# Wx-Alliance-Alliance-Meteo/paradis_model

Hardware: AMD Instinct MI355X
Metric: training samples/sec (whole node) on 5.625° ERA5 grid, 1/2/4/8 MI355X (higher is better)
Workload: dtype f32; 1 GPU; era5_5.625deg_32x64_S1_B32; grid=32x64, rollout_steps=1, per_gpu_batch=32, global_batch=32, parameters=60038475, optimizer=adamw, parallelism=dp1, gemm_arithmetic=bf16x3, mode=train, hip_graph=False, activation_checkpointing=False

## Files before the change

### paradis_model_amd/csrc/gemm_common.h

```cpp
#pragma once
#include <algorithm>
#include <cstdlib>
#include <initializer_list>
#include "common.h"

struct GemmArgs {
  const float* A; const float* B; float* C;
  int M, N, K;
  int64_t lda, ldb, ldc;
  int64_t a_bs, b_bs, c_bs;
  int nbatch;
  int inner;
  int64_t a_is, b_is;
  const float* bias; const float* map; const float* res; const float* zmul; float* zout;
  const float* gate;
  int64_t res_bs, zmul_bs, zout_bs;
  int act;
  int stagger;
  float* rowsum;
  const float* m8; const float* pw; int cin;
  const uint32_t* a_amax; const uint32_t* b_amax;
  int io16;
};

enum class WgradKind { Staged, Dma, Bf16x3, F16x2, Amp128, Tall, Square };
struct WgradWorkspace {
  int S, M, K;
  size_t rowsum_offset() const { return (size_t)S * M * K; }
  size_t bytes() const { return (size_t)S * M * ((size_t)K + 1) * sizeof(float) + 256; }
  float* rowsums(void* ws) const { return (float*)ws + rowsum_offset(); }
};

struct WgradPlan {
  WgradKind kind;
  int S;
  int grid, block;
  size_t lds;
  bool fused_rowsums;
  bool to_slabs;
  WgradWorkspace ws;
};

struct GemmTunables { int bk, wg_per_cu, stagger, dma_stages, wgrad_dma_stages; };
GemmTunables pd_exact_tunables();
int pd_exact_launch(bool a_kc, bool b_kc, const GemmArgs& g, int grid, hipStream_t st);
bool pd_exact_dma_eligible(const GemmArgs& g);
int pd_exact_launch_dma(const GemmArgs& g, int grid, hipStream_t st);
int pd_exact_launch_wgrad(const GemmArgs& g, const WgradPlan& p, hipStream_t st);
int pd_split_launch(const GemmArgs& d, int scheme, hipStream_t st);
int pd_split_launch_wgrad(const GemmArgs& g, const WgradPlan& p, hipStream_t st);
int64_t pd_split_image_chunks(int M, int K, int np);
void pd_split_launch_images(const float* A, int nbatch, int M, int K, int64_t a_bs, void* out, hipStream_t st);
int pd_amp_launch_fwd(const GemmArgs& d, hipStream_t st);
int pd_amp_launch_wgrad(const GemmArgs& g, int io16, const WgradPlan& p, hipStream_t st);

namespace {

typedef float f32x16 __attribute__((ext_vector_type(16)));

constexpr int BM = 128, BN = 128;

__device__ __forceinline__ void gemm_add_projection(const GemmArgs& g, f32x16 (&acc)[2][2], int m0, int n0,
                                                    int wm, int wn, int li, int lh) {
  const int nc0 = min(n0 + wn * 64 + li, g.N - 1), nc1 = min(n0 + wn * 64 + 32 + li, g.N - 1);
#pragma unroll 1
  for (int c = 0; c < g.cin; ++c) {
    const float mb0 = g.m8[(int64_t)c * g.N + nc0], mb1 = g.m8[(int64_t)c * g.N + nc1];
    const float* pc = g.pw + (int64_t)c * g.M;
#pragma unroll
    for (int tm = 0; tm < 2; ++tm) {
      const int mrow = m0 + wm * 64 + tm * 32 + 4 * lh;
#pragma unroll
      for (int j = 0; j < 4; ++j) {
        const int mr = mrow + 8 * j;
        const float4 p4 = (mr < g.M) ? *reinterpret_cast<const float4*>(pc + mr) : make_float4(0.f, 0.f, 0.f, 0.f);
        acc[tm][0][4 * j + 0] += p4.x * mb0; acc[tm][1][4 * j + 0] += p4.x * mb1;
        acc[tm][0][4 * j + 1] += p4.y * mb0; acc[tm][1][4 * j + 1] += p4.y * mb1;
        acc[tm][0][4 * j + 2] += p4.z * mb0; acc[tm][1][4 * j + 2] += p4.z * mb1;
        acc[tm][0][4 * j + 3] += p4.w * mb0; acc[tm][1][4 * j + 3] += p4.w * mb1;
      }
    }
  }
}

__device__ __forceinline__ float gate_sigmoid(float a) { return 1.0f / (1.0f + expf(-a)); }
__device__ __forceinline__ float round_bf16(float x) { return (float)(__bf16)x; }
__device__ __forceinline__ float sigmoid_r16(float z) {
  return __builtin_amdgcn_rcpf(1.0f + __builtin_amdgcn_exp2f(-1.44269504088896340736f * z));
}
__device__ __forceinline__ float act_apply_r16(float z, int act) {
  return act == PARADIS_ACT_SILU ? z * sigmoid_r16(z) : act_apply(z, act);
}
__device__ __forceinline__ float act_grad_r16(float z, int act) {
  if (act == PARADIS_ACT_SILU) {
    const float s = sigmoid_r16(z);
    return s * (1.0f + z * (1.0f - s));
  }
  return act_grad(z, act);
}
[[maybe_unused]] constexpr int IO_B16 = 1, IO_C16 = 2, IO_ZM16 = 4, IO_A16 = 8;
__device__ __forceinline__ float ld_bf16(const void* p, int64_t i) {
  return __uint_as_float((uint32_t)reinterpret_cast<const uint16_t*>(p)[i] << 16);
}
__device__ __forceinline__ void st_bf16(void* p, int64_t i, float v) {
  reinterpret_cast<uint16_t*>(p)[i] = (uint16_t)(__float_as_uint(v) >> 16);
}

template <bool R16 = false, bool C16 = false, bool ZM16 = false>
__device__ __forceinline__ void gemm_epilogue(const GemmArgs& g, f32x16 (&acc)[2][2], int bz, int m0,
                                              int n0, int wm, int wn, int li, int lh) {
  float* Cb = g.C + (int64_t)bz * g.c_bs;
  const float* resb = g.res ? g.res + (int64_t)bz * g.res_bs : nullptr;
  const float* zmulb = g.zmul ? g.zmul + (int64_t)bz * g.zmul_bs : nullptr;
  float* zoutb = g.zout ? g.zout + (int64_t)bz * g.zout_bs : nullptr;
  static_assert(R16 || !(C16 || ZM16), "bf16-stored tensors exist in the bf16-mixed scheme only");
  (void)sizeof(char[C16 + ZM16 + 1]);
  const int64_t cb16 = (int64_t)bz * g.c_bs, zmb16 = (int64_t)bz * g.zmul_bs, zob16 = (int64_t)bz * g.zout_bs;
  if (g.pw) gemm_add_projection(g, acc, m0, n0, wm, wn, li, lh);
  if constexpr (C16 || ZM16) {
    if (m0 + BM <= g.M && n0 + BN <= g.N && ((g.ldc | g.c_bs | g.zout_bs | g.zmul_bs) & 1) == 0) {
      const bool odd = (li & 1) != 0;
      const uint32_t sel = odd ? 0x07060302u : 0x03020706u;
      const int pcol = odd ? 31 + li : li;
      auto swap1 = [](float v) __attribute__((always_inline)) {
        return __int_as_float(__builtin_amdgcn_update_dpp(0, __float_as_int(v), 0xB1, 0xf, 0xf, false));
      };
      auto pack = [&](float a0, float a1) __attribute__((always_inline)) {
        const float keep = odd ? a1 : a0, recv = swap1(odd ? a0 : a1);
        return __builtin_amdgcn_perm(__float_as_uint(keep), __float_as_uint(recv), sel);
      };
      auto unpack = [&](uint32_t w, float& t0, float& t1) __attribute__((always_inline)) {
        const float wlo = __uint_as_float(w << 16), whi = __uint_as_float(w & 0xffff0000u);
        const float recv = swap1(odd ? wlo : whi);
        t0 = odd ? recv : wlo;
        t1 = odd ? whi : recv;
      };
#pragma unroll
      for (int tm = 0; tm < 2; ++tm) {
        const int mrow = m0 + wm * 64 + tm * 32 + 4 * lh;
        const int64_t base = (int64_t)mrow * g.ldc + n0 + wn * 64 + li;
        const int64_t pbase = (int64_t)mrow * g.ldc + n0 + wn * 64 + pcol;
#pragma unroll
        for (int h = 0; h < 4; ++h) {
          float v[2][4], t[2][4];
#define ROWOFF(q) ((int64_t)((q) + 8 * h) * g.ldc)
#pragma unroll
          for (int tn = 0; tn < 2; ++tn)
#pragma unroll
            for (int q = 0; q < 4; ++q) v[tn][q] = acc[tm][tn][4 * h + q];
          if (g.bias) {
#pragma unroll
            for (int q = 0; q < 4; ++q) t[0][q] = g.bias[mrow + q + 8 * h];
#pragma unroll
            for (int q = 0; q < 4; ++q) { v[0][q] += t[0][q]; v[1][q] += t[0][q]; }
          }
          if (g.map) {
#pragma unroll
            for (int tn = 0; tn < 2; ++tn)
#pragma unroll
              for (int q = 0; q < 4; ++q) t[tn][q] = g.map[base + 32 * tn + ROWOFF(q)];
#pragma unroll
            for (int tn = 0; tn < 2; ++tn)
#pragma unroll
              for (int q = 0; q < 4; ++q) v[tn][q] += t[tn][q];
          }
#pragma unroll
          for (int tn = 0; tn < 2; ++tn)
#pragma unroll
            for (int q = 0; q < 4; ++q) v[tn][q] = round_bf16(v[tn][q]);
          if (zoutb) {
            if constexpr (C16) {
#pragma unroll
              for (int q = 0; q < 4; ++q)
                reinterpret_cast<uint32_t*>(g.zout)[(zob16 + pbase + ROWOFF(q)) >> 1] = pack(v[0][q], v[1][q]);
            } else {
#pragma unroll
              for (int tn = 0; tn < 2; ++tn)
#pragma unroll
                for (int q = 0; q < 4; ++q) zoutb[base + 32 * tn + ROWOFF(q)] = v[tn][q];
            }
          }
          if (zmulb) {
            if constexpr (ZM16) {
              uint32_t w[4];
#pragma unroll
              for (int q = 0; q < 4; ++q) w[q] = reinterpret_cast<const uint32_t*>(g.zmul)[(zmb16 + pbase + ROWOFF(q)) >> 1];
#pragma unroll
              for (int q = 0; q < 4; ++q) unpack(w[q], t[0][q], t[1][q]);
            } else {
#pragma unroll
              for (int tn = 0; tn < 2; ++tn)
#pragma unroll
                for (int q = 0; q < 4; ++q) t[tn][q] = zmulb[base + 32 * tn + ROWOFF(q)];
            }
#pragma unroll
            for (int tn = 0; tn < 2; ++tn)
#pragma unroll
              for (int q = 0; q < 4; ++q) v[tn][q] *= act_grad_r16(t[tn][q], g.act);
          } else if (g.act) {
#pragma unroll
            for (int tn = 0; tn < 2; ++tn)
#pragma unroll
              for (int q = 0; q < 4; ++q) v[tn][q] = act_apply_r16(v[tn][q], g.act);
          }
          if (zmulb || g.act) {
#pragma unroll
            for (int tn = 0; tn < 2; ++tn)
#pragma unroll
              for (int q = 0; q < 4; ++q) v[tn][q] = round_bf16(v[tn][q]);
          }
          if (resb) {
#pragma unroll
            for (int tn = 0; tn < 2; ++tn)
#pragma unroll
              for (int q = 0; q < 4; ++q) t[tn][q] = resb[base + 32 * tn + ROWOFF(q)];
            if (g.gate) {
#pragma unroll
              for (int q = 0; q < 4; ++q) {
                const float gm = gate_sigmoid(g.gate[mrow + q + 8 * h]);
                v[0][q] = fmaf(gm, v[0][q] - t[0][q], t[0][q]);
                v[1][q] = fmaf(gm, v[1][q] - t[1][q], t[1][q]);
              }
            } else {
#pragma unroll
              for (int tn = 0; tn < 2; ++tn)
#pragma unroll
                for (int q = 0; q < 4; ++q) v[tn][q] += t[tn][q];
            }
          }
          if constexpr (C16) {
#pragma unroll
            for (int q = 0; q < 4; ++q)
              reinterpret_cast<uint32_t*>(g.C)[(cb16 + pbase + ROWOFF(q)) >> 1] = pack(v[0][q], v[1][q]);
          } else {
#pragma unroll
            for (int tn = 0; tn < 2; ++tn)
#pragma unroll
              for (int q = 0; q < 4; ++q) Cb[base + 32 * tn + ROWOFF(q)] = v[tn][q];
          }
          asm volatile("" ::: "memory");
          __builtin_amdgcn_sched_barrier(0);
#undef ROWOFF
        }
      }
      return;
    }
  }
  if (m0 + BM <= g.M && n0 + BN <= g.N) {
#pragma unroll
    for (int tm = 0; tm < 2; ++tm) {
      const int mrow = m0 + wm * 64 + tm * 32 + 4 * lh;
#pragma unroll
      for (int tn = 0; tn < 2; ++tn) {
        const int64_t base = (int64_t)mrow * g.ldc + n0 + wn * 64 + tn * 32 + li;
#pragma unroll
        for (int h = 0; h < 2; ++h) {
          float v[8], t[8];
#define ROWOFF(q) ((int64_t)(((q) & 3) + 8 * (2 * h + ((q) >> 2))) * g.ldc)
#pragma unroll
          for (int q = 0; q < 8; ++q) v[q] = acc[tm][tn][8 * h + q];
          if (g.bias) {
#pragma unroll
            for (int q = 0; q < 8; ++q) t[q] = g.bias[mrow + (q & 3) + 8 * (2 * h + (q >> 2))];
#pragma unroll
            for (int q = 0; q < 8; ++q) v[q] += t[q];
          }
          if (g.map) {
#pragma unroll
            for (int q = 0; q < 8; ++q) t[q] = g.map[base + ROWOFF(q)];
#pragma unroll
            for (int q = 0; q < 8; ++q) v[q] += t[q];
          }
          if constexpr (R16) {
#pragma unroll
            for (int q = 0; q < 8; ++q) v[q] = round_bf16(v[q]);
          }
          if (zoutb) {
            if constexpr (C16) {
#pragma unroll
              for (int q = 0; q < 8; ++q) st_bf16(g.zout, zob16 + base + ROWOFF(q), v[q]);
            } else {
#pragma unroll
              for (int q = 0; q < 8; ++q) zoutb[base + ROWOFF(q)] = v[q];
            }
          }
          if (zmulb) {
            if constexpr (ZM16) {
#pragma unroll
              for (int q = 0; q < 8; ++q) t[q] = ld_bf16(g.zmul, zmb16 + base + ROWOFF(q));
            } else {
#pragma unroll
              for (int q = 0; q < 8; ++q) t[q] = zmulb[base + ROWOFF(q)];
            }
#pragma unroll
            for (int q = 0; q < 8; ++q) v[q] *= R16 ? act_grad_r16(t[q], g.act) : act_grad(t[q], g.act);
          } else if (g.act) {
#pragma unroll
            for (int q = 0; q < 8; ++q) v[q] = R16 ? act_apply_r16(v[q], g.act) : act_apply(v[q], g.act);
          }
          if constexpr (R16) {
            if (zmulb || g.act) {
#pragma unroll
              for (int q = 0; q < 8; ++q) v[q] = round_bf16(v[q]);
            }
          }
          if (resb) {
#pragma unroll
            for (int q = 0; q < 8; ++q) t[q] = resb[base + ROWOFF(q)];
            if (g.gate) {
#pragma unroll
              for (int q = 0; q < 8; ++q) {
                const float gm = gate_sigmoid(g.gate[mrow + (q & 3) + 8 * (2 * h + (q >> 2))]);
                v[q] = fmaf(gm, v[q] - t[q], t[q]);
              }
            } else {
#pragma unroll
              for (int q = 0; q < 8; ++q) v[q] += t[q];
            }
          }
          if constexpr (C16) {
#pragma unroll
            for (int q = 0; q < 8; ++q) st_bf16(g.C, cb16 + base + ROWOFF(q), v[q]);
          } else {
#pragma unroll
            for (int q = 0; q < 8; ++q) Cb[base + ROWOFF(q)] = v[q];
          }
          asm volatile("" ::: "memory");
          __builtin_amdgcn_sched_barrier(0);
#undef ROWOFF
        }
      }
    }
    return;
  }
#pragma unroll
  for (int tm = 0; tm < 2; ++tm) {
#pragma unroll
    for (int r = 0; r < 16; ++r) {
      const int m = m0 + wm * 64 + tm * 32 + (r & 3) + 8 * (r >> 2) + 4 * lh;
      if (m >= g.M) continue;
      const float bv = g.bias ? g.bias[m] : 0.f;
#pragma unroll
      for (int tn = 0; tn < 2; ++tn) {
        const int n = n0 + wn * 64 + tn * 32 + li;
        if (n >= g.N) continue;
        const int64_t off = (int64_t)m * g.ldc + n;
        float v = acc[tm][tn][r] + bv;
        if (g.map) v += g.map[off];
        if constexpr (R16) v = round_bf16(v);
        if (zoutb) { if constexpr (C16) st_bf16(g.zout, zob16 + off, v); else zoutb[off] = v; }
        if (zmulb) {
          const float zm = ZM16 ? ld_bf16(g.zmul, zmb16 + off) : zmulb[off];
          v *= R16 ? act_grad_r16(zm, g.act) : act_grad(zm, g.act);
        } else if (g.act) {
          v = R16 ? act_apply_r16(v, g.act) : act_apply(v, g.act);
        }
        if constexpr (R16) { if (zmulb || g.act) v = round_bf16(v); }
        if (resb) {
          const float r = resb[off];
          v = g.gate ? fmaf(gate_sigmoid(g.gate[m]), v - r, r) : v + r;
        }
        if constexpr (C16) st_bf16(g.C, cb16 + off, v); else Cb[off] = v;
      }
    }
  }
}

typedef __attribute__((address_space(3))) void* lds_ptr_t;
typedef const __attribute__((address_space(1))) void* gbl_ptr_t;

typedef __bf16 bf16x8 __attribute__((ext_vector_type(8)));
typedef __bf16 bf16x2 __attribute__((ext_vector_type(2)));
typedef float f32x2 __attribute__((ext_vector_type(2)));
typedef uint32_t u32x4 __attribute__((ext_vector_type(4)));

constexpr int SBK = 16;
constexpr int SCH = 128;
constexpr int SCHP = 128 + 8;
constexpr int simg(int np) { return np * 2 * SCH; }
constexpr int simgp(int np) { return np * 2 * SCHP; }

#ifndef SPLIT_SIGNED
#define SPLIT_SIGNED 1
#endif
#ifndef SPLIT_SIGNED_WGRAD
#define SPLIT_SIGNED_WGRAD SPLIT_SIGNED
#endif
__device__ __forceinline__ uint32_t split_flip_mask(int col) { return SPLIT_SIGNED && (col & 64) ? 0x80000000u : 0u; }
__device__ __forceinline__ void flip8(float (&y)[8], const float (&x)[8], uint32_t mask) {
#pragma unroll
  for (int j = 0; j < 8; ++j) y[j] = __uint_as_float(__float_as_uint(x[j]) ^ mask);
}
__device__ __forceinline__ void split_unflip(f32x16 (&acc)[2][2], int wn) {
  if (!SPLIT_SIGNED) return;
  const float s0 = wn ? -1.f : 1.f, s1 = -s0;
#pragma unroll
  for (int tn = 0; tn < 2; ++tn)
#pragma unroll
    for (int r = 0; r < 16; ++r) { acc[0][tn][r] *= s0; acc[1][tn][r] *= s1; }
}

typedef _Float16 f16x8 __attribute__((ext_vector_type(8)));

__device__ __forceinline__ void scale_from_amax(uint32_t amax_bits, float& s, float& inv) {
  int E = (int)((amax_bits >> 23) & 0xffu);
  const bool finite = E != 255;
  E = E < 15 ? 15 : E;
  s = finite ? __uint_as_float((uint32_t)(268 - E) << 23) : __uint_as_float(0x7fc00000u);
  inv = __uint_as_float((uint32_t)(E - 14) << 23);
}

__device__ __forceinline__ uint32_t reduce_amax_partials(const uint32_t* __restrict__ p) {
  __shared__ uint32_t red[4];
  const int tid = threadIdx.x;
  uint32_t m = max(max(p[tid], p[tid + 256]), max(p[tid + 512], p[tid + 768]));
  m = wave_umax_lane63(m);
  if ((tid & 63) == 63) red[tid >> 6] = m;
  __syncthreads();
  m = max(max(red[0], red[1]), max(red[2], red[3]));
  __syncthreads();
  return m;
}

__device__ __forceinline__ void split2_pair(float x0, float x1, float s, uint32_t& h, uint32_t& l) {
  uint32_t hh, ll;
  asm("v_fma_mixlo_f16 %0, %1, %2, 0" : "=v"(hh) : "v"(x0), "v"(s));
  asm("v_fma_mixhi_f16 %0, %1, %2, 0" : "+v"(hh) : "v"(x1), "v"(s));
  asm("v_fma_mixlo_f16 %0, %1, %2, -%3 op_sel:[0,0,0] op_sel_hi:[0,0,1]" : "=v"(ll) : "v"(x0), "v"(s), "v"(hh));
  asm("v_fma_mixhi_f16 %0, %1, %2, -%3 op_sel:[0,0,1] op_sel_hi:[0,0,1]" : "+v"(ll) : "v"(x1), "v"(s), "v"(hh));
  h = hh; l = ll;
}

__device__ __forceinline__ uint32_t pack_bf16(float a, float b) {
  const f32x2 v = {a, b};
  return __builtin_bit_cast(uint32_t, __builtin_convertvector(v, bf16x2));
}

__device__ __forceinline__ void split_pair(float x0, float x1, uint32_t& h, uint32_t& m, uint32_t& l) {
  h = pack_bf16(x0, x1);
  const float r0 = x0 - __uint_as_float(h << 16), r1 = x1 - __uint_as_float(h & 0xffff0000u);
  m = pack_bf16(r0, r1);
  l = pack_bf16(r0 - __uint_as_float(m << 16), r1 - __uint_as_float(m & 0xffff0000u));
}

__device__ __forceinline__ void split8(const float (&x)[8], u32x4& h, u32x4& m, u32x4& l) {
  uint32_t hh[4], mm[4], ll[4];
#pragma unroll
  for (int i = 0; i < 4; ++i) split_pair(x[2 * i], x[2 * i + 1], hh[i], mm[i], ll[i]);
  h = (u32x4){hh[0], hh[1], hh[2], hh[3]};
  m = (u32x4){mm[0], mm[1], mm[2], mm[3]};
  l = (u32x4){ll[0], ll[1], ll[2], ll[3]};
}

__device__ __forceinline__ u32x4 round8(const float (&x)[8]) {
  return (u32x4){pack_bf16(x[0], x[1]), pack_bf16(x[2], x[3]), pack_bf16(x[4], x[5]), pack_bf16(x[6], x[7])};
}

__device__ __forceinline__ void split8_f16(const float (&x)[8], float s, u32x4& h, u32x4& l) {
  uint32_t hh[4], ll[4];
#pragma unroll
  for (int i = 0; i < 4; ++i) split2_pair(x[2 * i], x[2 * i + 1], s, hh[i], ll[i]);
  h = (u32x4){hh[0], hh[1], hh[2], hh[3]};
  l = (u32x4){ll[0], ll[1], ll[2], ll[3]};
}

#define SPLIT_MFMA(A, B, C) C = __builtin_amdgcn_mfma_f32_32x32x16_bf16(__builtin_bit_cast(bf16x8, A), __builtin_bit_cast(bf16x8, B), C, 0, 0, 0)
#define SPLIT_BLOCK(AH, AM, AL, BH, BM_, BL, C) \
  SPLIT_MFMA(AM, BM_, C); SPLIT_MFMA(AL, BH, C); SPLIT_MFMA(AH, BL, C); \
  SPLIT_MFMA(AM, BH, C);  SPLIT_MFMA(AH, BM_, C); SPLIT_MFMA(AH, BH, C)
#define SPLIT_MFMA16(A, B, C) C = __builtin_amdgcn_mfma_f32_32x32x16_f16(__builtin_bit_cast(f16x8, A), __builtin_bit_cast(f16x8, B), C, 0, 0, 0)

template <int NP> struct SplitFrags { u32x4 a[NP][2], b[NP][2]; };
template <int NP, int PA, int PB>
__device__ __forceinline__ void split_tile_read(const u32x4* As, const u32x4* Bs, SplitFrags<NP>& f) {
  if constexpr (NP == 3) {
    f.a[1][0] = As[PA];          f.b[1][0] = Bs[PB];
    f.a[2][0] = As[2 * PA];      f.b[0][0] = Bs[0];
    f.a[0][0] = As[0];           f.b[2][0] = Bs[2 * PB];
    f.b[1][1] = Bs[PB + 32];     f.b[0][1] = Bs[32];          f.b[2][1] = Bs[2 * PB + 32];
    f.a[1][1] = As[PA + 32];     f.a[2][1] = As[2 * PA + 32]; f.a[0][1] = As[32];
  } else if constexpr (NP == 2) {
    f.a[1][0] = As[PA];          f.b[0][0] = Bs[0];
    f.a[0][0] = As[0];           f.b[1][0] = Bs[PB];
    f.b[0][1] = Bs[32];          f.b[1][1] = Bs[PB + 32];
    f.a[1][1] = As[PA + 32];     f.a[0][1] = As[32];
  } else {
    f.a[0][0] = As[0];  f.b[0][0] = Bs[0];
    f.b[0][1] = Bs[32]; f.a[0][1] = As[32];
  }
}
template <int NP>
__device__ __forceinline__ void split_tile_mfma(const SplitFrags<NP>& f, f32x16 (&acc)[2][2]) {
#pragma unroll
  for (int tm = 0; tm < 2; ++tm)
#pragma unroll
    for (int tn = 0; tn < 2; ++tn) {
      if constexpr (NP == 3) {
        SPLIT_BLOCK(f.a[0][tm], f.a[1][tm], f.a[2][tm], f.b[0][tn], f.b[1][tn], f.b[2][tn], acc[tm][tn]);
      } else if constexpr (NP == 2) {
        SPLIT_MFMA16(f.a[1][tm], f.b[0][tn], acc[tm][tn]);
        SPLIT_MFMA16(f.a[0][tm], f.b[1][tn], acc[tm][tn]);
        SPLIT_MFMA16(f.a[0][tm], f.b[0][tn], acc[tm][tn]);
      } else {
        SPLIT_MFMA(f.a[0][tm], f.b[0][tn], acc[tm][tn]);
      }
    }
}

__device__ __forceinline__ void split_unscale(f32x16 (&acc)[2][2], float inv_a, float inv_b) {
#pragma unroll
  for (int i = 0; i < 2; ++i)
#pragma unroll
    for (int j = 0; j < 2; ++j)
#pragma unroll
      for (int r = 0; r < 16; ++r) acc[i][j][r] = (acc[i][j][r] * inv_a) * inv_b;
}

typedef float f32x4 __attribute__((ext_vector_type(4)));
template <int NP>
__global__ void __launch_bounds__(256, 3)
pw_gemm_wgrad_split_kernel(GemmArgs g) {
  extern __shared__ __attribute__((aligned(16))) float lds[];
  constexpr int SIMGP = simgp(NP);
  u32x4* img = reinterpret_cast<u32x4*>(lds);
  const int tid = threadIdx.x, lane = tid & 63, wave = tid >> 6;
  const int wm = wave >> 1, wn = wave & 1;
  const int li = lane & 31, lh = lane >> 5;

  const int MT = (g.M + BM - 1) / BM, NT = (g.N + BN - 1) / BN;
  int L;
  {
    const int nwg = gridDim.x, id = blockIdx.x;
    const int q = nwg >> 3, r = nwg & 7, xcd = id & 7;
    L = (xcd < r ? xcd * (q + 1) : r * (q + 1) + (xcd - r) * q) + (id >> 3);
  }
  const int mt = L % MT, nt = (L / MT) % NT, bz = L / (MT * NT);
  const int m0 = mt * BM, n0 = nt * BN;
  const int KT = g.K / SBK;
  const int64_t total = (int64_t)g.inner * KT;
  const int t_begin = (int)(total * bz / g.nbatch);
  const int T = (int)(total * (bz + 1) / g.nbatch) - t_begin;

  const int srow = tid >> 1, sh = tid & 1;
  const float* Ag = g.A + (int64_t)min(m0 + srow, g.M - 1) * g.lda + sh * 8;
  const float* Bg = g.B + (int64_t)min(n0 + srow, g.N - 1) * g.ldb + sh * 8;

  int f_ib = t_begin / KT, f_kt = t_begin - f_ib * KT;
  struct Regs { f32x4 a0, a1, b0, b1; };
  const f32x4 zero4 = {0.f, 0.f, 0.f, 0.f};
  Regs r0{zero4, zero4, zero4, zero4}, r1 = r0;
  auto fetch = [&](Regs& r) __attribute__((always_inline)) {
    const float* a = Ag + (int64_t)f_ib * g.a_is + (int64_t)f_kt * SBK;
    const float* b = Bg + (int64_t)f_ib * g.b_is + (int64_t)f_kt * SBK;
    asm volatile("global_load_dwordx4 %0, %1, off" : "=&v"(r.a0) : "v"(a) : "memory");
    asm volatile("global_load_dwordx4 %0, %1, off offset:16" : "=&v"(r.a1) : "v"(a) : "memory");
    asm volatile("global_load_dwordx4 %0, %1, off" : "=&v"(r.b0) : "v"(b) : "memory");
    asm volatile("global_load_dwordx4 %0, %1, off offset:16" : "=&v"(r.b1) : "v"(b) : "memory");
    if (++f_kt == KT) { f_kt = 0; ++f_ib; }
  };
#define USE_R(r, N) do { asm volatile("s_waitcnt vmcnt(" #N ")" :: "v"(r.a0), "v"(r.a1), "v"(r.b0), "v"(r.b1) : "memory"); \
                         __builtin_amdgcn_sched_barrier(0); } while (0)
  const bool do_rowsum = g.rowsum != nullptr && nt == 0;
  float rs = 0.f;
  float sc_a = 1.f, sc_b = 1.f, inv_a = 1.f, inv_b = 1.f;
  if constexpr (NP == 2) {
    scale_from_amax(reduce_amax_partials(g.a_amax), sc_a, inv_a);
    scale_from_amax(reduce_amax_partials(g.b_amax), sc_b, inv_b);
  }
  const uint32_t slab_flip = (SPLIT_SIGNED_WGRAD && (bz & 1)) ? 0x80000000u : 0u;
  if constexpr (NP == 2) sc_a = __uint_as_float(__float_as_uint(sc_a) ^ slab_flip);
  auto split_store = [&](const Regs& r, int st, bool keep) __attribute__((always_inline)) {
    const float xa[8] = {r.a0.x, r.a0.y, r.a0.z, r.a0.w, r.a1.x, r.a1.y, r.a1.z, r.a1.w};
    const float xb[8] = {r.b0.x, r.b0.y, r.b0.z, r.b0.w, r.b1.x, r.b1.y, r.b1.z, r.b1.w};
    const float add = ((xa[0] + xa[1]) + (xa[2] + xa[3])) + ((xa[4] + xa[5]) + (xa[6] + xa[7]));
    rs += keep ? add : 0.f;
    u32x4* o = img + st * 2 * SIMGP + sh * SCHP + srow;
    if constexpr (NP == 3) {
      u32x4 ha, ma, la, hb, mb, lb;
      float xs[8];
      flip8(xs, xa, slab_flip);
      split8(xs, ha, ma, la);
      split8(xb, hb, mb, lb);
      o[0] = ha; o[2 * SCHP] = ma; o[4 * SCHP] = la;
      o += SIMGP;
      o[0] = hb; o[2 * SCHP] = mb; o[4 * SCHP] = lb;
    } else if constexpr (NP == 1) {
      float xs[8];
      flip8(xs, xa, slab_flip);
      o[0] = round8(xs);
      o[SIMGP] = round8(xb);
    } else {
      u32x4 ha, la, hb, lb;
      split8_f16(xa, sc_a, ha, la);
      split8_f16(xb, sc_b, hb, lb);
      o[0] = ha; o[2 * SCHP] = la;
      o += SIMGP;
      o[0] = hb; o[2 * SCHP] = lb;
    }
  };

  f32x16 acc[2][2];
#pragma unroll
  for (int i = 0; i < 2; ++i)
#pragma unroll
    for (int j = 0; j < 2; ++j)
#pragma unroll
      for (int r = 0; r < 16; ++r) acc[i][j][r] = 0.f;

  if (T > 0) {
    fetch(r0);
    if (T > 1) { fetch(r1); USE_R(r0, 4); } else { USE_R(r0, 0); }
    split_store(r0, 0, do_rowsum);
  }
  asm volatile("s_waitcnt lgkmcnt(0)\n\ts_barrier" ::: "memory");

  auto step = [&](int t, int cur, Regs& rload, Regs& rsplit) __attribute__((always_inline)) {
    const u32x4* As = img + cur * 2 * SIMGP + lh * SCHP + wm * 64 + li;
    const u32x4* Bs = img + (cur * 2 + 1) * SIMGP + lh * SCHP + wn * 64 + li;
    SplitFrags<NP> f;
    split_tile_read<NP, 2 * SCHP, 2 * SCHP>(As, Bs, f);
    __builtin_amdgcn_sched_barrier(0);
    if (t + 2 < T) { fetch(rload); USE_R(rsplit, 4); }
    else USE_R(rsplit, 0);
    split_tile_mfma<NP>(f, acc);
    split_store(rsplit, cur ^ 1, do_rowsum && t + 1 < T);
    if constexpr (NP > 1) {
#pragma unroll
    for (int i = 0; i < (NP == 3 ? 24 : 12); ++i) {
      __builtin_amdgcn_sched_group_barrier(0x008, 1, 0);
      __builtin_amdgcn_sched_group_barrier(0x002, 5, 0);
    }
    }
    asm volatile("s_waitcnt lgkmcnt(0)\n\ts_barrier" ::: "memory");
  };
  for (int t = 0; t < T; t += 2) {
    step(t, 0, r0, r1);
    if (t + 1 < T) step(t + 1, 1, r1, r0);
  }
#undef USE_R
  if (do_rowsum) {
    rs += __shfl_xor(rs, 1, 64);
    const int m = m0 + srow;
    if (sh == 0 && m < g.M) g.rowsum[(int64_t)bz * g.M + m] = rs;
  }
  if (slab_flip) {
#pragma unroll
    for (int i = 0; i < 2; ++i)
#pragma unroll
      for (int j = 0; j < 2; ++j)
#pragma unroll
        for (int r = 0; r < 16; ++r) acc[i][j][r] = -acc[i][j][r];
  }
  if constexpr (NP == 2) split_unscale(acc, inv_a, inv_b);
  gemm_epilogue(g, acc, bz, m0, n0, wm, wn, li, lh);
}

typedef void (*GemmKernel)(GemmArgs);
#define IO2_KERNELS(K) {&K<false, false>, &K<true, false>, &K<false, true>, &K<true, true>}

inline int reserve_lds(GemmKernel k, size_t bytes, const char* what) {
  if (hipFuncSetAttribute(reinterpret_cast<const void*>(k), hipFuncAttributeMaxDynamicSharedMemorySize, (int)bytes) == hipSuccess) return 0;
  paradis_set_error("%s: cannot reserve LDS", what);
  return 2;
}
inline int reserve_lds(PerDeviceOnce& once, std::initializer_list<GemmKernel> ks, size_t bytes, const char* what) {
  if (!once.first()) return 0;
  for (GemmKernel k : ks)
    if (int e = reserve_lds(k, bytes, what)) return e;
  return 0;
}

template <const GemmKernel (&KS)[4]>
int launch_io2(bool a, bool b, dim3 grid, dim3 block, size_t lds, const char* reserve_for, hipStream_t st, const GemmArgs& g) {
  static PerDeviceOnce once;
  if (reserve_for)
    if (int e = reserve_lds(once, {KS[0], KS[1], KS[2], KS[3]}, lds, reserve_for)) return e;
  hipLaunchKernelGGL(KS[a + 2 * b], grid, block, lds, st, g);
  return 0;
}

struct GemmKernelEntry { GemmKernel k; size_t lds; };
template <int N>
int reserve_lds(PerDeviceOnce& once, const GemmKernelEntry (&tab)[N], const char* what) {
  bool any = false;
  for (const GemmKernelEntry& e : tab) any = any || (e.k && e.lds > 64 * 1024);
  if (!any || !once.first()) return 0;
  for (const GemmKernelEntry& e : tab)
    if (e.k && e.lds > 64 * 1024)
      if (int err = reserve_lds(e.k, e.lds, what)) return err;
  return 0;
}
template <int N>
int launch_entry(const GemmKernelEntry (&tab)[N], int i, PerDeviceOnce& once, const char* what, int grid, int block,
                 hipStream_t st, const GemmArgs& g, size_t lds = 0) {
  if (i < 0 || i >= N || tab[i].k == nullptr) { paradis_set_error("%s: no kernel for index %d", what, i); return 1; }
  if (int e = reserve_lds(once, tab, what)) return e;
  hipLaunchKernelGGL(tab[i].k, dim3(grid), dim3(block), lds ? lds : tab[i].lds, st, g);
  return 0;
}

constexpr int DBK = 16;
constexpr int DTILE = DBK * BM;
constexpr size_t dma_lds_bytes(int stages) { return (size_t)stages * 2 * DTILE * sizeof(float); }
constexpr int stage_floats(int bk) { return bk * (BM + 4); }
constexpr size_t lds_bytes(int bk) { return (size_t)4 * stage_floats(bk) * sizeof(float); }
constexpr size_t STAGED_LDS_MAX = 160 * 1024;
inline size_t staged_lds_request(int bk, int wg_per_cu) {
  return std::min(std::max(lds_bytes(bk), (size_t)(160 * 1024 / wg_per_cu) & ~(size_t)255), STAGED_LDS_MAX);
}
constexpr size_t split_lds_wgrad(int np) { return (size_t)2 * 2 * simgp(np) * 16; }
constexpr int TALL_PA = 256 + 8, TALL_PB = 128 + 8, TALL_STAGE = 2 * TALL_PA + 2 * TALL_PB;
constexpr size_t tall_lds_bytes() { return (size_t)2 * TALL_STAGE * 16; }
constexpr int SQ_P = 256 + 8, SQ_STAGE = 4 * SQ_P;
constexpr size_t sq_lds_bytes() { return (size_t)4 * SQ_STAGE * 16; }


struct WgradEnv { bool tall, square; };
inline WgradEnv wgrad_env() {
  static const WgradEnv env = [] {
    const char *t = getenv("PARADIS_WGRAD_TALL"), *s = getenv("PARADIS_WGRAD_SQUARE");
    return WgradEnv{!(t && t[0] == '0'), !(s && s[0] == '0')};
  }();
  return env;
}

struct WgradTile { int th, tw, kd, wg_per_cu, block; size_t lds; };
inline WgradTile wgrad_tile(WgradKind kind, const GemmTunables& t) {
  switch (kind) {
    case WgradKind::Staged: return {BM, BN, t.bk, t.wg_per_cu, 256, staged_lds_request(t.bk, t.wg_per_cu)};
    case WgradKind::Dma:    return {BM, BN, DBK, t.wgrad_dma_stages == 2 ? 4 : 3, 256, dma_lds_bytes(t.wgrad_dma_stages)};
    case WgradKind::Bf16x3: return {BM, BN, SBK, 3, 256, split_lds_wgrad(3)};
    case WgradKind::F16x2:  return {BM, BN, SBK, 3, 256, split_lds_wgrad(2)};
    case WgradKind::Amp128: return {BM, BN, SBK, 3, 256, split_lds_wgrad(1)};
    case WgradKind::Tall:   return {256, BN, SBK, 2, 512, tall_lds_bytes()};
    case WgradKind::Square: return {256, 256, SBK, 1, 512, sq_lds_bytes()};
  }
  return {};
}
constexpr WgradKind WGRAD_KINDS[] = {WgradKind::Staged, WgradKind::Dma,  WgradKind::Bf16x3, WgradKind::F16x2,
                                     WgradKind::Amp128, WgradKind::Tall, WgradKind::Square};

inline int wgrad_splits(int B, int M, int K, int N, const WgradTile& tl) {
  const int tiles = ((M + tl.th - 1) / tl.th) * ((K + tl.tw - 1) / tl.tw);
  const int64_t total_kt = (int64_t)B * ((N + tl.kd - 1) / tl.kd);
  int s = (int)std::max<int64_t>(1, std::min<int64_t>(256 * tl.wg_per_cu / tiles, total_kt));
  if (s > 1) s &= ~1;
  return s;
}

inline bool wgrad_fills_256(int n) { return ((n + 255) / 256) * 256 * 7 <= n * 8; }

inline WgradKind wgrad_kind(int M, int K, int N, int64_t dy_bs, int64_t x_bs, const void* dY, const void* X, int scheme,
                            int io16, const GemmTunables& t, WgradEnv env) {
  const bool vec = N % DBK == 0 && (dy_bs & 3) == 0 && (x_bs & 3) == 0 && aligned16(dY) && aligned16(X);
  if (io16 != 0 || (scheme != PARADIS_GEMM_EXACT && vec)) {
    if (scheme == PARADIS_GEMM_BF16) {
      const bool tall = env.tall && M >= 256 && wgrad_fills_256(M);
      return tall && env.square && wgrad_fills_256(K) ? WgradKind::Square : tall ? WgradKind::Tall : WgradKind::Amp128;
    }
    return scheme == PARADIS_GEMM_F16X2 ? WgradKind::F16x2 : WgradKind::Bf16x3;
  }
  return t.wgrad_dma_stages >= 2 && vec ? WgradKind::Dma : WgradKind::Staged;
}

inline WgradPlan wgrad_plan_of(WgradKind kind, int B, int M, int K, int N, const GemmTunables& t) {
  const WgradTile tl = wgrad_tile(kind, t);
  const int S = wgrad_splits(B, M, K, N, tl), grid = ((M + tl.th - 1) / tl.th) * ((K + tl.tw - 1) / tl.tw) * S;
  return {kind, S, grid, tl.block, tl.lds, kind != WgradKind::Staged, S > 1, {S, M, K}};
}

inline WgradPlan wgrad_plan(int B, int M, int K, int N, int64_t dy_bs, int64_t x_bs, const void* dY, const void* X, int scheme,
                            int io16, const GemmTunables& t, WgradEnv env) {
  return wgrad_plan_of(wgrad_kind(M, K, N, dy_bs, x_bs, dY, X, scheme, io16, t, env), B, M, K, N, t);
}

inline size_t wgrad_ws_bytes(int B, int M, int K, int N, const GemmTunables& t) {
  size_t bytes = 0;
  for (WgradKind kind : WGRAD_KINDS) bytes = std::max(bytes, wgrad_plan_of(kind, std::max(B, 1), M, K, N, t).ws.bytes());
  return bytes;
}

struct SlabReduce { int64_t n; int vec, blocks1, n2, blocks2; };
inline SlabReduce wgrad_reduce(const WgradPlan& p, const void* workspace, const void* dW, bool rowsums) {
  const int64_t n = p.to_slabs ? (int64_t)p.ws.M * p.ws.K : 0;
  const int vec = n % 4 == 0 && aligned16(workspace) && aligned16(dW);
  const int n2 = rowsums ? p.ws.M : 0;
  return {n, vec, n ? (int)std::min<int64_t>(((vec ? n / 4 : n) + 255) / 256, 2048) : 0, n2, (n2 + 255) / 256};
}
}
```

### paradis_model_amd/csrc/gemm_split.hip

```cpp
#include <cstring>
#include <type_traits>
#include "gemm_common.h"

namespace {

constexpr int SIMG = simg(3);

__global__ void __launch_bounds__(256)
amax_partials_kernel(const float* __restrict__ x, int B, int64_t inner, int64_t bs, int vec, uint32_t* __restrict__ out) {
  uint32_t m = 0;
  if (vec) {
    const int64_t n4 = inner >> 2, total = n4 * B;
    for (int64_t i = (int64_t)blockIdx.x * 256 + threadIdx.x; i < total; i += (int64_t)gridDim.x * 256) {
      const int64_t b = i / n4, j = i - b * n4;
      const uint4 q = *reinterpret_cast<const uint4*>(x + b * bs + 4 * j);
      m = max(max(m, q.x & 0x7fffffffu), max(q.y & 0x7fffffffu, max(q.z & 0x7fffffffu, q.w & 0x7fffffffu)));
    }
  } else {
    const int64_t total = inner * B;
    for (int64_t i = (int64_t)blockIdx.x * 256 + threadIdx.x; i < total; i += (int64_t)gridDim.x * 256) {
      const int64_t b = i / inner, j = i - b * inner;
      m = max(m, __float_as_uint(x[b * bs + j]) & 0x7fffffffu);
    }
  }
  m = wave_umax_lane63(m);
  __shared__ uint32_t red[4];
  if ((threadIdx.x & 63) == 63) red[threadIdx.x >> 6] = m;
  __syncthreads();
  if (threadIdx.x == 0) out[blockIdx.x] = max(max(red[0], red[1]), max(red[2], red[3]));
}


template <int NP = 3>
__device__ __forceinline__ void split_weights_body(const float* __restrict__ Wb, int64_t rs, int64_t cs, int M, int K,
                                                   int KT, int64_t units, u32x4* __restrict__ ob) {
  for (int64_t u = (int64_t)blockIdx.x * 256 + threadIdx.x; u < units; u += (int64_t)gridDim.x * 256) {
    const int row = (int)(u & 127), half = (int)((u >> 7) & 1);
    const int64_t tile = u >> 8;
    const int kt = (int)(tile % KT), mt = (int)(tile / KT);
    const int m = mt * BM + row;
    float x[8];
#pragma unroll
    for (int j = 0; j < 8; ++j) {
      const int k = kt * SBK + half * 8 + j;
      x[j] = (m < M && k < K) ? Wb[(int64_t)m * rs + (int64_t)k * cs] : 0.f;
      if (SPLIT_SIGNED && (row & 32)) x[j] = -x[j];
    }
    if constexpr (NP == 3) {
      u32x4 h, mm, l;
      split8(x, h, mm, l);
      u32x4* o = ob + tile * SIMG + half * SCH + row;
      o[0] = h; o[2 * SCH] = mm; o[4 * SCH] = l;
    } else {
      ob[tile * simg(1) + half * SCH + row] = round8(x);
    }
  }
}

template <int NP>
__global__ void __launch_bounds__(256)
split_weights_kernel(const float* __restrict__ W, int64_t rs, int64_t cs, int M, int K, int KT, int64_t units,
                     int64_t w_bs, int64_t out_bs, u32x4* __restrict__ out) {
  split_weights_body<NP>(W + (int64_t)blockIdx.y * w_bs, rs, cs, M, K, KT, units, out + (int64_t)blockIdx.y * out_bs);
}

template <int NP>
__global__ void __launch_bounds__(256)
split_weights_pair_kernel(const float* __restrict__ W, int M, int K, int KT, int KTt, int64_t units, int64_t units_t,
                          u32x4* __restrict__ out, u32x4* __restrict__ out_t) {
  if (blockIdx.y == 0) split_weights_body<NP>(W, K, 1, M, K, KT, units, out);
  else split_weights_body<NP>(W, 1, K, K, M, KTt, units_t, out_t);
}

__global__ void __launch_bounds__(256)
split_weights_f16_kernel(const float* __restrict__ W, int64_t rs, int64_t cs, int M, int K, int KT, int64_t units,
                         u32x4* __restrict__ out, uint32_t* __restrict__ tail) {
  const uint32_t amax = reduce_amax_partials(tail + 4);
  if (blockIdx.x == 0 && threadIdx.x == 0) tail[0] = amax;
  float sc, inv;
  scale_from_amax(amax, sc, inv);
  for (int64_t u = (int64_t)blockIdx.x * 256 + threadIdx.x; u < units; u += (int64_t)gridDim.x * 256) {
    const int row = (int)(u & 127), half = (int)((u >> 7) & 1);
    const int64_t tile = u >> 8;
    const int kt = (int)(tile % KT), mt = (int)(tile / KT);
    const int m = mt * BM + row;
    float x[8];
#pragma unroll
    for (int j = 0; j < 8; ++j) {
      const int k = kt * SBK + half * 8 + j;
      x[j] = (m < M && k < K) ? W[(int64_t)m * rs + (int64_t)k * cs] : 0.f;
    }
    u32x4 h, l;
    split8_f16(x, (SPLIT_SIGNED && (row & 32)) ? -sc : sc, h, l);
    u32x4* o = out + tile * simg(2) + half * SCH + row;
    o[0] = h; o[2 * SCH] = l;
  }
}

enum : int { EP_ON = 1, EP_BIAS = 2, EP_MAP = 4, EP_ZOUT = 8, EP_SILU = 16, EP_ZMUL = 32, EP_RES = 64, EP_GATE = 128 };

template <int OFF>
__device__ __forceinline__ void ep_load(float& x, uint32_t voff, const float* p) {
  asm volatile("global_load_dword %0, %1, %2 offset:%3" : "=&v"(x) : "v"(voff), "s"(p), "n"(OFF) : "memory");
}
template <int OFF>
__device__ __forceinline__ void ep_store(float x, uint32_t voff, float* p) {
  asm volatile("global_store_dword %0, %1, %2 offset:%3" :: "v"(voff), "v"(x), "s"(p), "n"(OFF) : "memory");
}
template <int N>
__device__ __forceinline__ void ep_wait(const float (&a)[8]) {
  asm volatile("s_waitcnt vmcnt(%0)" :: "n"(N), "v"(a[0]), "v"(a[1]), "v"(a[2]), "v"(a[3]), "v"(a[4]), "v"(a[5]), "v"(a[6]),
               "v"(a[7]) : "memory");
  __builtin_amdgcn_sched_barrier(0);
}
template <int N>
__device__ __forceinline__ void ep_wait(const float (&a)[8], const float (&b)[8]) {
  asm volatile("s_waitcnt vmcnt(%0)" :: "n"(N), "v"(a[0]), "v"(a[1]), "v"(a[2]), "v"(a[3]), "v"(a[4]), "v"(a[5]), "v"(a[6]),
               "v"(a[7]), "v"(b[0]), "v"(b[1]), "v"(b[2]), "v"(b[3]), "v"(b[4]), "v"(b[5]), "v"(b[6]), "v"(b[7]) : "memory");
  __builtin_amdgcn_sched_barrier(0);
}
template <int N>
__device__ __forceinline__ void ep_wait(float a, float b) {
  asm volatile("s_waitcnt vmcnt(%0)" :: "n"(N), "v"(a), "v"(b) : "memory");
  __builtin_amdgcn_sched_barrier(0);
}
__device__ __forceinline__ float ep_row(float rowvec, int addr) {
  return __int_as_float(__builtin_amdgcn_ds_bpermute(addr, __float_as_int(rowvec)));
}
template <class T>
__device__ __forceinline__ T* ep_uniform(T* p) {
  const uint64_t a = reinterpret_cast<uint64_t>(p);
  const uint32_t lo = __builtin_amdgcn_readfirstlane((uint32_t)a), hi = __builtin_amdgcn_readfirstlane((uint32_t)(a >> 32));
  return reinterpret_cast<T*>(((uint64_t)hi << 32) | lo);
}

template <int EPI>
__device__ __forceinline__ void split_epilogue_interior(const GemmArgs& g, f32x16 (&acc)[2][2], int bz, int m0, int n0,
                                                        int wm, int wn, int li, int lh) {
  constexpr bool BIAS = EPI & EP_BIAS, MAP = EPI & EP_MAP, ZOUT = EPI & EP_ZOUT, SILU = EPI & EP_SILU, ZMUL = EPI & EP_ZMUL,
                 RES = EPI & EP_RES, GATE = EPI & EP_GATE;
  static_assert(!(GATE && !RES) && !(ZMUL && (SILU || ZOUT)), "no such epilogue");
  constexpr int NT = MAP + ZMUL + RES, I_MAP = 0, I_ZM = MAP, I_RES = MAP + ZMUL;
  static_assert(NT <= 2, "a third operand tensor needs a third ep_wait");
  constexpr int L = 8 * NT, S = 8 * (1 + ZOUT);
  const int wrow = __builtin_amdgcn_readfirstlane(m0 + wm * 64), wcol = __builtin_amdgcn_readfirstlane(n0 + wn * 64);
  const int64_t ld = g.ldc, tile = (int64_t)wrow * ld + wcol;
  float* const Cs = ep_uniform(g.C + (int64_t)bz * g.c_bs + tile);
  float* const zos = ZOUT ? ep_uniform(g.zout + (int64_t)bz * g.zout_bs + tile) : nullptr;
  const float* const mps = MAP ? ep_uniform(g.map + tile) : nullptr;
  const float* const zms = ZMUL ? ep_uniform(g.zmul + (int64_t)bz * g.zmul_bs + tile) : nullptr;
  const float* const rss = RES ? ep_uniform(g.res + (int64_t)bz * g.res_bs + tile) : nullptr;
  const uint32_t voff = ((uint32_t)(4 * lh) * (uint32_t)ld + (uint32_t)li) * 4u;
  const int radr = 16 * lh;
  auto rowof = [](int gi, int q) constexpr { return (gi >> 2) * 32 + (q & 3) + 8 * (2 * ((gi >> 1) & 1) + (q >> 2)); };

  float bv = 0.f, gv = 0.f;
  float buf[2][NT ? NT : 1][8];
  auto issue = [&](auto G) __attribute__((always_inline)) {
    constexpr int gi = decltype(G)::value, OFF = (gi & 1) * 128;
#pragma unroll
    for (int q = 0; q < 8; ++q) {
      const int64_t ro = (int64_t)rowof(gi, q) * ld;
      if constexpr (MAP) ep_load<OFF>(buf[gi & 1][I_MAP][q], voff, mps + ro);
      if constexpr (ZMUL) ep_load<OFF>(buf[gi & 1][I_ZM][q], voff, zms + ro);
      if constexpr (RES) ep_load<OFF>(buf[gi & 1][I_RES][q], voff, rss + ro);
    }
  };
  float br[8], gr[8];
  if constexpr (BIAS) ep_load<0>(bv, (uint32_t)(32 * lh + li) * 4u, ep_uniform(g.bias + wrow));
  if constexpr (GATE) ep_load<0>(gv, (uint32_t)(32 * lh + li) * 4u, ep_uniform(g.gate + wrow));
  if constexpr (NT > 0) issue(std::integral_constant<int, 0>{});
  __builtin_amdgcn_sched_barrier(0);

  auto group = [&](auto G) __attribute__((always_inline)) {
    constexpr int gi = decltype(G)::value, tm = gi >> 2, h = (gi >> 1) & 1, tn = gi & 1, OFF = tn * 128, b = gi & 1;
    if constexpr (NT > 0 && gi < 7) {
      issue(std::integral_constant<int, gi + 1>{});
      __builtin_amdgcn_sched_barrier(0);
    }
    if constexpr (gi == 0 && (BIAS || GATE)) {
      ep_wait<NT ? 2 * L : 0>(bv, gv);
      if constexpr (GATE) gv = gate_sigmoid(gv);
    }
    if constexpr (tn == 0 && (BIAS || GATE)) {
#pragma unroll
      for (int q = 0; q < 8; ++q) {
        if constexpr (BIAS) br[q] = ep_row(bv, radr + 4 * rowof(gi, q));
        if constexpr (GATE) gr[q] = ep_row(gv, radr + 4 * rowof(gi, q));
      }
      __builtin_amdgcn_sched_barrier(0);
    }
    constexpr int YOUNGER = (gi < 7 ? L : 0) + (gi > 0 ? S : 0);
    if constexpr (NT == 1) ep_wait<YOUNGER>(buf[b][0]);
    if constexpr (NT == 2) ep_wait<YOUNGER>(buf[b][0], buf[b][1]);
    float v[8];
#pragma unroll
    for (int q = 0; q < 8; ++q) v[q] = acc[tm][tn][8 * h + q];
    if constexpr (BIAS) {
#pragma unroll
      for (int q = 0; q < 8; ++q) v[q] += br[q];
    }
    if constexpr (MAP) {
#pragma unroll
      for (int q = 0; q < 8; ++q) v[q] += buf[b][I_MAP][q];
    }
    if constexpr (ZOUT) {
#pragma unroll
      for (int q = 0; q < 8; ++q) ep_store<OFF>(v[q], voff, zos + (int64_t)rowof(gi, q) * ld);
    }
    if constexpr (ZMUL) {
#pragma unroll
      for (int q = 0; q < 8; ++q) v[q] *= act_grad(buf[b][I_ZM][q], PARADIS_ACT_SILU);
    } else if constexpr (SILU) {
#pragma unroll
      for (int q = 0; q < 8; ++q) v[q] = act_apply(v[q], PARADIS_ACT_SILU);
    }
    if constexpr (RES) {
#pragma unroll
      for (int q = 0; q < 8; ++q) {
        const float r = buf[b][I_RES][q];
        if constexpr (GATE) v[q] = fmaf(gr[q], v[q] - r, r);
        else v[q] += r;
      }
    }
#pragma unroll
    for (int q = 0; q < 8; ++q) ep_store<OFF>(v[q], voff, Cs + (int64_t)rowof(gi, q) * ld);
    __builtin_amdgcn_sched_barrier(0);
  };
  group(std::integral_constant<int, 0>{}); group(std::integral_constant<int, 1>{});
  group(std::integral_constant<int, 2>{}); group(std::integral_constant<int, 3>{});
  group(std::integral_constant<int, 4>{}); group(std::integral_constant<int, 5>{});
  group(std::integral_constant<int, 6>{}); group(std::integral_constant<int, 7>{});
}

#ifndef SPLIT_ASTAGES_F16
#define SPLIT_ASTAGES_F16 2
#endif
constexpr int split_astages(int np) { return np == 2 ? SPLIT_ASTAGES_F16 : 2; }
template <int NP>
__global__ void __launch_bounds__(256, 3)
pw_gemm_split_kernel(GemmArgs g) {
  extern __shared__ __attribute__((aligned(16))) float lds[];
  constexpr int SIMG = simg(NP);
  u32x4* img = reinterpret_cast<u32x4*>(lds);
  constexpr int SA = split_astages(NP), DA = SA - 1;
  const int tid = threadIdx.x, lane = tid & 63, wave = tid >> 6;
  const int wm = wave >> 1, wn = wave & 1;
  const int li = lane & 31, lh = lane >> 5;

  const int MT = (g.M + BM - 1) / BM, NT = (g.N + BN - 1) / BN;
  int L;
  {
    const int nwg = gridDim.x, id = blockIdx.x;
    const int q = nwg >> 3, r = nwg & 7, xcd = id & 7;
    L = (xcd < r ? xcd * (q + 1) : r * (q + 1) + (xcd - r) * q) + (id >> 3);
  }
  const int mt = L % MT, nt = (L / MT) % NT, bz = L / (MT * NT);
  const int m0 = mt * BM, n0 = nt * BN;
  const int T = (g.K + SBK - 1) / SBK;

  const u32x4* Ag = reinterpret_cast<const u32x4*>(g.A) + (int64_t)bz * g.a_bs + (int64_t)mt * T * SIMG + tid;
  const int bh = __builtin_amdgcn_readfirstlane(tid >> 7);
  const float* Bb;
  {
    const uint64_t a = reinterpret_cast<uint64_t>(g.B + (int64_t)bz * g.b_bs);
    const uint32_t lo = __builtin_amdgcn_readfirstlane((uint32_t)a), hi = __builtin_amdgcn_readfirstlane((uint32_t)(a >> 32));
    Bb = reinterpret_cast<const float*>(((uint64_t)hi << 32) | lo);
  }
  const int bn = min(n0 + (tid & 127), g.N - 1);

  float sc_b = 1.f, inv_a = 1.f, inv_b = 1.f;
  if constexpr (NP == 2) {
    float sc_a;
    scale_from_amax(reduce_amax_partials(g.b_amax), sc_b, inv_b);
    scale_from_amax(g.a_amax[0], sc_a, inv_a);
  }

  const uint32_t flip = split_flip_mask(tid & 127);
  if constexpr (NP == 2) sc_b = __uint_as_float(__float_as_uint(sc_b) ^ flip);
  float xb[2][8] = {};
  auto issueA = [&](int t) __attribute__((always_inline)) {
    const u32x4* a = Ag + (int64_t)t * SIMG;
    u32x4* la = img + (2 + t % SA) * SIMG + wave * 64;
#pragma unroll
    for (int i = 0; i < NP; ++i)
      __builtin_amdgcn_global_load_lds((gbl_ptr_t)(a + i * 256), (lds_ptr_t)(la + i * 256), 16, 0, 0);
  };
  auto split_store = [&](const float (&x)[8], u32x4* o) __attribute__((always_inline)) {
    if constexpr (NP == 3) {
      u32x4 h, m, l;
      float xs[8];
      flip8(xs, x, flip);
      split8(xs, h, m, l);
      o[0] = h; o[2 * SCH] = m; o[4 * SCH] = l;
    } else {
      u32x4 h, l;
      split8_f16(x, sc_b, h, l);
      o[0] = h; o[2 * SCH] = l;
    }
  };
  const uint32_t boff = (uint32_t)bn * 4u;
  auto fetchB = [&](int t, float (&x)[8]) __attribute__((always_inline)) {
    const int k0 = t * SBK + bh * 8;
    const float* p = Bb + (int64_t)min(k0, g.K - 1) * g.ldb;
#pragma unroll
    for (int j = 0; j < 8; ++j) {
      asm volatile("global_load_dword %0, %1, %2" : "=&v"(x[j]) : "v"(boff), "s"(p) : "memory");
      p += (k0 + j + 1 < g.K) ? g.ldb : 0;
    }
  };
#define USE_X(x, N) do { asm volatile("s_waitcnt vmcnt(" #N ")" :: "v"(x[0]), "v"(x[1]), "v"(x[2]), "v"(x[3]), \
                                      "v"(x[4]), "v"(x[5]), "v"(x[6]), "v"(x[7]) : "memory");                  \
                         __builtin_amdgcn_sched_barrier(0); } while (0)
  u32x4* const Bst = img + bh * SCH + (tid & 127);

  f32x16 acc[2][2];
#pragma unroll
  for (int i = 0; i < 2; ++i)
#pragma unroll
    for (int j = 0; j < 2; ++j)
#pragma unroll
      for (int r = 0; r < 16; ++r) acc[i][j][r] = 0.f;

  for (int u = 0; u < DA && u < T; ++u) issueA(u);
  fetchB(0, xb[0]);
  USE_X(xb[0], 0);
  if (T > 1) fetchB(1, xb[1]);
  split_store(xb[0], Bst);
  if (T > 1) asm volatile("s_waitcnt vmcnt(8) lgkmcnt(0)\n\ts_barrier" ::: "memory");
  else asm volatile("s_waitcnt vmcnt(0) lgkmcnt(0)\n\ts_barrier" ::: "memory");
  auto step = [&](int t, int cur, float (&xload)[8], float (&xsplit)[8]) __attribute__((always_inline)) {
    const u32x4* As = img + (2 + t % SA) * SIMG + lh * SCH + wm * 64 + li;
    const u32x4* Bs = img + cur * SIMG + lh * SCH + wn * 64 + li;
    const bool dmaA = t + DA < T, ldB = t + 2 < T;
    if (dmaA) issueA(t + DA);
    if (ldB) fetchB(t + 2, xload);
    if (dmaA && ldB) { if constexpr (NP == 3) USE_X(xsplit, 11); else USE_X(xsplit, 10); }
    else if (ldB) USE_X(xsplit, 8);
    else USE_X(xsplit, 0);
    SplitFrags<NP> f;
    split_tile_read<NP, 2 * SCH, 2 * SCH>(As, Bs, f);
    split_tile_mfma<NP>(f, acc);
    split_store(xsplit, Bst + (cur ^ 1) * SIMG);
    __builtin_amdgcn_sched_group_barrier(0x100, 4 * NP, 0);
#pragma unroll
    for (int i = 0; i < (NP == 3 ? 24 : 12); ++i) {
      __builtin_amdgcn_sched_group_barrier(0x008, 1, 0);
      __builtin_amdgcn_sched_group_barrier(0x002, NP == 3 ? 3 : 2, 0);
    }
    if (dmaA && ldB) asm volatile("s_waitcnt vmcnt(%0) lgkmcnt(0)\n\ts_barrier" :: "n"(8 + (8 + NP) * (DA - 1)) : "memory");
    else asm volatile("s_waitcnt vmcnt(0) lgkmcnt(0)\n\ts_barrier" ::: "memory");
  };
  for (int t = 0; t < T; t += 2) {
    step(t, 0, xb[0], xb[1]);
    if (t + 1 < T) step(t + 1, 1, xb[1], xb[0]);
  }
  split_unflip(acc, wn);
  if constexpr (NP == 2) split_unscale(acc, inv_a, inv_b);
  gemm_epilogue(g, acc, bz, m0, n0, wm, wn, li, lh);
}

#ifndef SPLIT_STAGGER
#define SPLIT_STAGGER 0
#endif
template <int NSUB, int NP = 2, int EPI = 0>
__global__ void __launch_bounds__(256 * NSUB, 4)
pw_gemm_split_wide_kernel(GemmArgs g) {
  extern __shared__ __attribute__((aligned(16))) float lds[];
  constexpr int SIMG = simg(NP), SA = 2, DA = SA - 1;
  u32x4* img = reinterpret_cast<u32x4*>(lds);
  const int tid = threadIdx.x, lane = tid & 63, wave = tid >> 6;
  const int sub = __builtin_amdgcn_readfirstlane(wave >> 2), lw = wave & 3, ltid = tid & 255;
  const int wm = lw >> 1, wn = lw & 1;
  const int li = lane & 31, lh = lane >> 5;

  const int MT = (g.M + BM - 1) / BM, NT = (g.N + BN - 1) / BN, NT2 = (NT + NSUB - 1) / NSUB;
  int L;
  {
    const int nwg = gridDim.x, id = blockIdx.x;
    const int q = nwg >> 3, r = nwg & 7, xcd = id & 7;
    L = (xcd < r ? xcd * (q + 1) : r * (q + 1) + (xcd - r) * q) + (id >> 3);
  }
  const int mt = L % MT, nt2 = (L / MT) % NT2, bz = L / (MT * NT2);
  const bool live = NSUB * nt2 + sub < NT;
  const int nt = min(NSUB * nt2 + sub, NT - 1);
  const int m0 = mt * BM, n0 = nt * BN;
  const int T = (g.K + SBK - 1) / SBK;

  const bool doA = NSUB == 2 || wave < 8;
  const bool doA2 = NP == 3 && wave < 4;
  const u32x4* Ag = reinterpret_cast<const u32x4*>(g.A) + (int64_t)bz * g.a_bs + (int64_t)mt * T * SIMG + (tid & 511);
  const int bh = __builtin_amdgcn_readfirstlane(ltid >> 7);
  const float* Bb;
  {
    const uint64_t a = reinterpret_cast<uint64_t>(g.B + (int64_t)bz * g.b_bs);
    const uint32_t lo = __builtin_amdgcn_readfirstlane((uint32_t)a), hi = __builtin_amdgcn_readfirstlane((uint32_t)(a >> 32));
    Bb = reinterpret_cast<const float*>(((uint64_t)hi << 32) | lo);
  }
  const int bn = min(n0 + (ltid & 127), g.N - 1);

  float sc_b = 1.f, inv_a = 1.f, inv_b = 1.f;
  if constexpr (NP == 2) {
    float sc_a;
    __shared__ uint32_t red[4 * NSUB];
    const uint32_t* pp = g.b_amax;
    uint32_t m = NSUB == 2 ? max(pp[tid], pp[tid + 512]) : pp[tid];
    m = wave_umax_lane63(m);
    if (lane == 63) red[wave] = m;
    __syncthreads();
    m = red[0];
#pragma unroll
    for (int i = 1; i < 4 * NSUB; ++i) m = max(m, red[i]);
    scale_from_amax(m, sc_b, inv_b);
    scale_from_amax(g.a_amax[0], sc_a, inv_a);
  }

  const uint32_t flip = split_flip_mask(ltid & 127);
  if constexpr (NP == 2) sc_b = __uint_as_float(__float_as_uint(sc_b) ^ flip);
  float xb[2][8] = {};
  auto issueA = [&](int t) __attribute__((always_inline)) {
    if (doA)
      __builtin_amdgcn_global_load_lds((gbl_ptr_t)(Ag + (int64_t)t * SIMG), (lds_ptr_t)(img + (2 * NSUB + t % SA) * SIMG + wave * 64), 16, 0, 0);
    if (doA2)
      __builtin_amdgcn_global_load_lds((gbl_ptr_t)(Ag + (int64_t)t * SIMG + 512), (lds_ptr_t)(img + (2 * NSUB + t % SA) * SIMG + 512 + wave * 64), 16, 0, 0);
  };
  auto split_store = [&](const float (&x)[8], u32x4* o) __attribute__((always_inline)) {
    if constexpr (NP == 3) {
      u32x4 h, m, l;
      float xs[8];
      flip8(xs, x, flip);
      split8(xs, h, m, l);
      o[0] = h; o[2 * SCH] = m; o[4 * SCH] = l;
    } else {
      u32x4 h, l;
      split8_f16(x, sc_b, h, l);
      o[0] = h; o[2 * SCH] = l;
    }
  };
  const uint32_t boff = (uint32_t)bn * 4u;
  auto fetchB = [&](int t, float (&x)[8]) __attribute__((always_inline)) {
    const int k0 = t * SBK + bh * 8;
    const float* p = Bb + (int64_t)min(k0, g.K - 1) * g.ldb;
#pragma unroll
    for (int j = 0; j < 8; ++j) {
      asm volatile("global_load_dword %0, %1, %2" : "=&v"(x[j]) : "v"(boff), "s"(p) : "memory");
      p += (k0 + j + 1 < g.K) ? g.ldb : 0;
    }
  };
#define USE_X(x, N) do { asm volatile("s_waitcnt vmcnt(" #N ")" :: "v"(x[0]), "v"(x[1]), "v"(x[2]), "v"(x[3]), \
                                      "v"(x[4]), "v"(x[5]), "v"(x[6]), "v"(x[7]) : "memory");                  \
                         __builtin_amdgcn_sched_barrier(0); } while (0)
  u32x4* const Bst = img + sub * 2 * SIMG + bh * SCH + (ltid & 127);

  f32x16 acc[2][2];
#pragma unroll
  for (int i = 0; i < 2; ++i)
#pragma unroll
    for (int j = 0; j < 2; ++j)
#pragma unroll
      for (int r = 0; r < 16; ++r) acc[i][j][r] = 0.f;

  for (int u = 0; u < DA && u < T; ++u) issueA(u);
  fetchB(0, xb[0]);
  USE_X(xb[0], 0);
  if (T > 1) fetchB(1, xb[1]);
  split_store(xb[0], Bst);
  if (T > 1) asm volatile("s_waitcnt vmcnt(8) lgkmcnt(0)\n\ts_barrier" ::: "memory");
  else asm volatile("s_waitcnt vmcnt(0) lgkmcnt(0)\n\ts_barrier" ::: "memory");
  auto step = [&](int t, int cur, float (&xload)[8], float (&xsplit)[8]) __attribute__((always_inline)) {
    const u32x4* As = img + (2 * NSUB + t % SA) * SIMG + lh * SCH + wm * 64 + li;
    const u32x4* Bs = img + (sub * 2 + cur) * SIMG + lh * SCH + wn * 64 + li;
    const bool dmaA = t + DA < T, ldB = t + 2 < T;
    if (dmaA) issueA(t + DA);
    if (ldB) fetchB(t + 2, xload);
    if (dmaA && ldB && doA2) USE_X(xsplit, 10);
    else if (dmaA && ldB && doA) USE_X(xsplit, 9);
    else if (ldB) USE_X(xsplit, 8);
    else USE_X(xsplit, 0);
    if constexpr (NP == 3) {
      auto mfma_block = [&]() __attribute__((always_inline)) {
        u32x4 a[3][2], b[2];
#pragma unroll
        for (int pl = 0; pl < 3; ++pl) { a[pl][0] = As[pl * 2 * SCH]; a[pl][1] = As[pl * 2 * SCH + 32]; }
#pragma unroll
        for (int pb = 2; pb >= 0; --pb) {
          b[0] = Bs[pb * 2 * SCH]; b[1] = Bs[pb * 2 * SCH + 32];
#pragma unroll
          for (int pa = 2 - pb; pa >= 0; --pa)
#pragma unroll
            for (int tm = 0; tm < 2; ++tm)
#pragma unroll
              for (int tn = 0; tn < 2; ++tn) SPLIT_MFMA(a[pa][tm], b[tn], acc[tm][tn]);
        }
      };
#if SPLIT_STAGGER
      if (sub == 1) split_store(xsplit, Bst + (cur ^ 1) * SIMG);
      __builtin_amdgcn_sched_barrier(0);
      mfma_block();
      __builtin_amdgcn_sched_barrier(0);
      if (sub == 0) split_store(xsplit, Bst + (cur ^ 1) * SIMG);
#else
      mfma_block();
      split_store(xsplit, Bst + (cur ^ 1) * SIMG);
#endif
    } else {
      SplitFrags<NP> f;
      split_tile_read<NP, 2 * SCH, 2 * SCH>(As, Bs, f);
      split_tile_mfma<NP>(f, acc);
      split_store(xsplit, Bst + (cur ^ 1) * SIMG);
      __builtin_amdgcn_sched_group_barrier(0x100, 4 * NP, 0);
#pragma unroll
      for (int i = 0; i < 12; ++i) {
        __builtin_amdgcn_sched_group_barrier(0x008, 1, 0);
        __builtin_amdgcn_sched_group_barrier(0x002, 2, 0);
      }
    }
    if (dmaA && ldB) asm volatile("s_waitcnt vmcnt(8) lgkmcnt(0)\n\ts_barrier" ::: "memory");
    else asm volatile("s_waitcnt vmcnt(0) lgkmcnt(0)\n\ts_barrier" ::: "memory");
  };
  for (int t = 0; t < T; t += 2) {
    step(t, 0, xb[0], xb[1]);
    if (t + 1 < T) step(t + 1, 1, xb[1], xb[0]);
  }
#undef USE_X
  if (live) {
    if constexpr (EPI != 0) {
      int t = tid;
      asm volatile("" : "+v"(t));
      const int ew = __builtin_amdgcn_readfirstlane((t >> 6) & 3), ewm = ew >> 1, ewn = ew & 1, eli = t & 31, elh = (t >> 5) & 1;
      split_unflip(acc, ewn);
      if constexpr (NP == 2) split_unscale(acc, inv_a, inv_b);
      if (m0 + BM <= g.M && n0 + BN <= g.N) split_epilogue_interior<EPI>(g, acc, bz, m0, n0, ewm, ewn, eli, elh);
      else gemm_epilogue(g, acc, bz, m0, n0, ewm, ewn, eli, elh);
    } else {
      split_unflip(acc, wn);
      if constexpr (NP == 2) split_unscale(acc, inv_a, inv_b);
      gemm_epilogue(g, acc, bz, m0, n0, wm, wn, li, lh);
    }
  }
}


constexpr size_t split_lds(int np) { return (size_t)(2 + split_astages(np)) * simg(np) * 16; }
constexpr int AMAX_WORDS = PARADIS_AMAX_PARTIALS;
constexpr size_t F16_TAIL_BYTES = 16 + (size_t)AMAX_WORDS * 4;

int split_image_ktiles(int K, int np) {
  const int kt = (K + SBK - 1) / SBK;
  return np == 1 ? (kt + 1) & ~1 : kt;
}
int64_t split_image_chunks(int M, int K, int np = 3) {
  return (int64_t)((M + BM - 1) / BM) * split_image_ktiles(K, np) * simg(np);
}

int launch_amax(const float* x, int B, int64_t inner, int64_t bs, uint32_t* out, hipStream_t st) {
  const int vec = (inner % 4 == 0) && (bs % 4 == 0) && aligned16(x);
  hipLaunchKernelGGL(amax_partials_kernel, dim3(AMAX_WORDS), dim3(256), 0, st, x, B, inner, bs, vec, out);
  return 0;
}

constexpr size_t split_wide_lds(int nsub, int np = 2) { return (size_t)(2 * nsub + 2) * simg(np) * 16; }
constexpr int SPLIT_WIDE_NSUB = 2;
#ifndef SPLIT_WIDE_BF16X3
#define SPLIT_WIDE_BF16X3 1
#endif
constexpr GemmKernelEntry SPLIT[2] = {{&pw_gemm_split_kernel<2>, split_lds(2)}, {&pw_gemm_split_kernel<3>, split_lds(3)}};
constexpr GemmKernelEntry SPLIT_WIDE[2] = {{&pw_gemm_split_wide_kernel<SPLIT_WIDE_NSUB, 2>, split_wide_lds(SPLIT_WIDE_NSUB, 2)},
                                           {&pw_gemm_split_wide_kernel<SPLIT_WIDE_NSUB, 3>, split_wide_lds(SPLIT_WIDE_NSUB, 3)}};
constexpr GemmKernelEntry SPLIT_WGRAD[2] = {{&pw_gemm_wgrad_split_kernel<2>, split_lds_wgrad(2)},
                                            {&pw_gemm_wgrad_split_kernel<3>, split_lds_wgrad(3)}};
#define EPI_SETS(X)                                                                                                       \
  X(EP_ON) X(EP_ON | EP_ZMUL)                                                                         \
  X(EP_ON | EP_BIAS) X(EP_ON | EP_BIAS | EP_RES) X(EP_ON | EP_BIAS | EP_RES | EP_GATE)                      \
  X(EP_ON | EP_BIAS | EP_SILU | EP_ZOUT) X(EP_ON | EP_BIAS | EP_MAP | EP_RES)                                            \
  X(EP_ON | EP_BIAS | EP_MAP | EP_SILU | EP_ZOUT)
#define EPI_SET(E) (E),
#define EPI_ENTRY(E) {&pw_gemm_split_wide_kernel<SPLIT_WIDE_NSUB, 3, (E)>, split_wide_lds(SPLIT_WIDE_NSUB, 3)},
constexpr int SPLIT_WIDE_EPI_SETS[] = {EPI_SETS(EPI_SET)};
constexpr GemmKernelEntry SPLIT_WIDE_EPI[] = {EPI_SETS(EPI_ENTRY)};
#undef EPI_ENTRY
#undef EPI_SET
#undef EPI_SETS

int split_epilogue_flags(const GemmArgs& d) {
  const char* e = getenv("PARADIS_GEMM_EPILOGUE");
  if (e && strcmp(e, "generic") == 0) return 0;
  if (d.pw || d.io16 || d.ldc >= (1 << 26) || (d.gate && !d.res)) return 0;
  if (d.zmul ? d.act != PARADIS_ACT_SILU : (d.act != 0 && d.act != PARADIS_ACT_SILU)) return 0;
  return EP_ON | (d.bias ? EP_BIAS : 0) | (d.map ? EP_MAP : 0) | (d.zout ? EP_ZOUT : 0) | (d.zmul ? EP_ZMUL : 0) |
         (!d.zmul && d.act ? EP_SILU : 0) | (d.res ? EP_RES : 0) | (d.gate ? EP_GATE : 0);
}

}

extern "C" size_t paradis_pw_gemm_split_bytes(int M, int K, int scheme) {
  if (M < 1 || K < 1) return 0;
  if (scheme == PARADIS_GEMM_F16X2) return (size_t)split_image_chunks(M, K, 2) * 16 + F16_TAIL_BYTES;
  if (scheme == PARADIS_GEMM_BF16) return (size_t)split_image_chunks(M, K, 1) * 16;
  return scheme == PARADIS_GEMM_BF16X3 ? (size_t)split_image_chunks(M, K, 3) * 16 : 0;
}

extern "C" int paradis_amax_partials(const float* x, int B, int64_t inner, int64_t bs, uint32_t* partials,
                                     void* stream) {
  PD_REQUIRE(partials != nullptr && B >= 0 && inner >= 0 && (x != nullptr || B == 0 || inner == 0),
             "amax_partials: bad arguments");
  launch_amax(x, B, inner, bs, partials, (hipStream_t)stream);
  PD_CHECK_LAUNCH("amax_partials");
  return 0;
}

extern "C" int paradis_pw_gemm_split_weights(const float* W, int M, int K, int transpose, int scheme, void* out,
                                             void* stream) {
  PD_REQUIRE(W != nullptr && out != nullptr && M >= 1 && K >= 1, "pw_gemm_split_weights: bad arguments");
  PD_REQUIRE(scheme == PARADIS_GEMM_BF16X3 || scheme == PARADIS_GEMM_F16X2 || scheme == PARADIS_GEMM_BF16,
             "pw_gemm_split_weights: unknown scheme %d", scheme);
  const int AM = transpose ? K : M, AK = transpose ? M : K;
  const int KT = split_image_ktiles(AK, scheme == PARADIS_GEMM_BF16 ? 1 : 3);
  const int64_t units = (int64_t)((AM + BM - 1) / BM) * KT * 256;
  const int blocks = (int)std::min<int64_t>((units + 255) / 256, 4096);
  if (scheme == PARADIS_GEMM_F16X2) {
    uint32_t* tail = reinterpret_cast<uint32_t*>((char*)out + (size_t)split_image_chunks(AM, AK, 2) * 16);
    launch_amax(W, 1, (int64_t)M * K, 0, tail + 4, (hipStream_t)stream);
    hipLaunchKernelGGL(split_weights_f16_kernel, dim3(blocks), dim3(256), 0, (hipStream_t)stream, W,
                       (int64_t)(transpose ? 1 : K), (int64_t)(transpose ? K : 1), AM, AK, KT, units, (u32x4*)out, tail);
  } else if (scheme == PARADIS_GEMM_BF16) {
    hipLaunchKernelGGL(split_weights_kernel<1>, dim3(blocks, 1), dim3(256), 0, (hipStream_t)stream, W,
                       (int64_t)(transpose ? 1 : K), (int64_t)(transpose ? K : 1), AM, AK, KT, units,
                       (int64_t)0, (int64_t)0, (u32x4*)out);
  } else {
    hipLaunchKernelGGL(split_weights_kernel<3>, dim3(blocks, 1), dim3(256), 0, (hipStream_t)stream, W,
                       (int64_t)(transpose ? 1 : K), (int64_t)(transpose ? K : 1), AM, AK, KT, units,
                       (int64_t)0, (int64_t)0, (u32x4*)out);
  }
  PD_CHECK_LAUNCH("pw_gemm_split_weights");
  return 0;
}

extern "C" int paradis_pw_gemm_split_weights_pair_scheme(const float* W, int M, int K, int scheme, void* out, void* out_t,
                                                         void* stream) {
  PD_REQUIRE(W != nullptr && out != nullptr && out_t != nullptr && out != out_t && M >= 1 && K >= 1,
             "pw_gemm_split_weights_pair: bad arguments");
  PD_REQUIRE(scheme == PARADIS_GEMM_BF16X3 || scheme == PARADIS_GEMM_BF16,
             "pw_gemm_split_weights_pair: scheme %d has no paired images", scheme);
  const int np = scheme == PARADIS_GEMM_BF16 ? 1 : 3;
  const int KT = split_image_ktiles(K, np), KTt = split_image_ktiles(M, np);
  const int64_t units = (int64_t)((M + BM - 1) / BM) * KT * 256, units_t = (int64_t)((K + BM - 1) / BM) * KTt * 256;
  const int blocks = (int)std::min<int64_t>((std::max(units, units_t) + 255) / 256, 4096);
  if (scheme == PARADIS_GEMM_BF16X3)
    hipLaunchKernelGGL(split_weights_pair_kernel<3>, dim3(blocks, 2), dim3(256), 0, (hipStream_t)stream, W, M, K, KT, KTt,
                       units, units_t, (u32x4*)out, (u32x4*)out_t);
  else
    hipLaunchKernelGGL(split_weights_pair_kernel<1>, dim3(blocks, 2), dim3(256), 0, (hipStream_t)stream, W, M, K, KT, KTt,
                       units, units_t, (u32x4*)out, (u32x4*)out_t);
  PD_CHECK_LAUNCH("pw_gemm_split_weights_pair");
  return 0;
}
extern "C" int paradis_pw_gemm_split_weights_pair(const float* W, int M, int K, void* out, void* out_t, void* stream) {
  return paradis_pw_gemm_split_weights_pair_scheme(W, M, K, PARADIS_GEMM_BF16X3, out, out_t, stream);
}


int pd_split_launch(const GemmArgs& d, int scheme, hipStream_t st) {
  static PerDeviceOnce once, once_wide, once_epi;
  const int np = scheme == PARADIS_GEMM_F16X2 ? 2 : 3;
  const int MT = (d.M + BM - 1) / BM, NT = (d.N + BN - 1) / BN;
  if (NT >= 2 && np == 3 && SPLIT_WIDE_BF16X3) {
    constexpr int NE = sizeof(SPLIT_WIDE_EPI_SETS) / sizeof(int);
    const int set = split_epilogue_flags(d);
    for (int i = 0; set != 0 && i < NE; ++i)
      if (SPLIT_WIDE_EPI_SETS[i] == set)
        return launch_entry(SPLIT_WIDE_EPI, i, once_epi, "pw_gemm(split)", MT * ((NT + SPLIT_WIDE_NSUB - 1) / SPLIT_WIDE_NSUB) * d.nbatch,
                            256 * SPLIT_WIDE_NSUB, st, d);
  }
  if (NT >= 2 && (np == 2 || SPLIT_WIDE_BF16X3))
    return launch_entry(SPLIT_WIDE, np - 2, once_wide, "pw_gemm(split)", MT * ((NT + SPLIT_WIDE_NSUB - 1) / SPLIT_WIDE_NSUB) * d.nbatch,
                        256 * SPLIT_WIDE_NSUB, st, d);
  return launch_entry(SPLIT, np - 2, once, "pw_gemm(split)", MT * NT * d.nbatch, 256, st, d);
}

int pd_split_launch_wgrad(const GemmArgs& g, const WgradPlan& p, hipStream_t st) {
  static PerDeviceOnce once;
  return launch_entry(SPLIT_WGRAD, p.kind == WgradKind::F16x2 ? 0 : 1, once, "pw_gemm_wgrad(split)", p.grid, p.block, st, g, p.lds);
}

int64_t pd_split_image_chunks(int M, int K, int np) { return split_image_chunks(M, K, np); }

void pd_split_launch_images(const float* A, int nbatch, int M, int K, int64_t a_bs, void* out, hipStream_t st) {
  const int KT = (K + SBK - 1) / SBK;
  const int64_t units = (int64_t)((M + BM - 1) / BM) * KT * 256;
  const int blocks = (int)std::min<int64_t>((units + 255) / 256, 1024);
  hipLaunchKernelGGL(split_weights_kernel<3>, dim3(blocks, nbatch), dim3(256), 0, st, A, (int64_t)K, (int64_t)1, M, K, KT, units,
                     a_bs, split_image_chunks(M, K), (u32x4*)out);
}
```

Before: 214.1 samples/s.

## Specialize split GEMM loops per sign/rowsum and use scalar-base loads in wgrad

Each bf16x3 split GEMM main loop now runs as a compile-time specialization chosen by the wave-uniform sign flip. Negation is folded into the bf16 pack instruction, so the per-element flip8 XOR disappears. Rowsum accumulation is specialized out of the loop, and a wgrad variant uses SGPR base plus 32-bit VGPR offset loads when leading dimensions fit. The goal is fewer VALU ops and VGPRs in the hot loop, at the cost of code size and more instantiations. A new generic_epilogue flag and a templated interior epilogue with pipelined loads are also added.

```diff
diff --git a/paradis_model_amd/csrc/gemm_common.h b/paradis_model_amd/csrc/gemm_common.h
--- a/paradis_model_amd/csrc/gemm_common.h
+++ b/paradis_model_amd/csrc/gemm_common.h
@@ -2,6 +2,7 @@
 #include <algorithm>
 #include <cstdlib>
 #include <initializer_list>
+#include <type_traits>
 #include "common.h"
 
 struct GemmArgs {
@@ -18,6 +19,7 @@
   int act;
   int stagger;
   float* rowsum;
+  int generic_epilogue;
   const float* m8; const float* pw; int cin;
   const uint32_t* a_amax; const uint32_t* b_amax;
   int io16;
@@ -386,6 +388,24 @@
 #ifndef SPLIT_SIGNED_WGRAD
 #define SPLIT_SIGNED_WGRAD SPLIT_SIGNED
 #endif
+#ifndef SPLIT_SIGN_LOOPS
+#define SPLIT_SIGN_LOOPS 1
+#endif
+#ifndef SPLIT_SIGN_LOOPS_FWD
+#define SPLIT_SIGN_LOOPS_FWD SPLIT_SIGN_LOOPS
+#endif
+#ifndef SPLIT_SIGN_LOOPS_WGRAD
+#define SPLIT_SIGN_LOOPS_WGRAD SPLIT_SIGN_LOOPS
+#endif
+#ifndef SPLIT_WGRAD_ROWSUM_LOOP
+#define SPLIT_WGRAD_ROWSUM_LOOP SPLIT_SIGN_LOOPS
+#endif
+#ifndef SPLIT_WGRAD_SADDR
+#define SPLIT_WGRAD_SADDR SPLIT_SIGN_LOOPS
+#endif
+#ifndef SPLIT_WGRAD_EPILOGUE
+#define SPLIT_WGRAD_EPILOGUE SPLIT_SIGN_LOOPS
+#endif
 __device__ __forceinline__ uint32_t split_flip_mask(int col) { return SPLIT_SIGNED && (col & 64) ? 0x80000000u : 0u; }
 __device__ __forceinline__ void flip8(float (&y)[8], const float (&x)[8], uint32_t mask) {
 #pragma unroll
@@ -450,6 +470,26 @@
   h = (u32x4){hh[0], hh[1], hh[2], hh[3]};
   m = (u32x4){mm[0], mm[1], mm[2], mm[3]};
   l = (u32x4){ll[0], ll[1], ll[2], ll[3]};
+}
+
+template <bool FLIP>
+__device__ __forceinline__ void split8s(const float (&x)[8], u32x4& h, u32x4& m, u32x4& l) {
+  if constexpr (!FLIP) {
+    split8(x, h, m, l);
+  } else {
+    uint32_t hh[4], mm[4], ll[4];
+#pragma unroll
+    for (int i = 0; i < 4; ++i) {
+      const float x0 = x[2 * i], x1 = x[2 * i + 1];
+      asm("v_cvt_pk_bf16_f32 %0, -%1, -%2" : "=v"(hh[i]) : "v"(x0), "v"(x1));
+      const float r0 = (-x0) - __uint_as_float(hh[i] << 16), r1 = (-x1) - __uint_as_float(hh[i] & 0xffff0000u);
+      mm[i] = pack_bf16(r0, r1);
+      ll[i] = pack_bf16(r0 - __uint_as_float(mm[i] << 16), r1 - __uint_as_float(mm[i] & 0xffff0000u));
+    }
+    h = (u32x4){hh[0], hh[1], hh[2], hh[3]};
+    m = (u32x4){mm[0], mm[1], mm[2], mm[3]};
+    l = (u32x4){ll[0], ll[1], ll[2], ll[3]};
+  }
 }
 
 __device__ __forceinline__ u32x4 round8(const float (&x)[8]) {
@@ -516,11 +556,151 @@
       for (int r = 0; r < 16; ++r) acc[i][j][r] = (acc[i][j][r] * inv_a) * inv_b;
 }
 
+enum : int { EP_ON = 1, EP_BIAS = 2, EP_MAP = 4, EP_ZOUT = 8, EP_SILU = 16, EP_ZMUL = 32, EP_RES = 64, EP_GATE = 128 };
+
+template <int OFF>
+__device__ __forceinline__ void ep_load(float& x, uint32_t voff, const float* p) {
+  asm volatile("global_load_dword %0, %1, %2 offset:%3" : "=&v"(x) : "v"(voff), "s"(p), "n"(OFF) : "memory");
+}
+template <int OFF>
+__device__ __forceinline__ void ep_store(float x, uint32_t voff, float* p) {
+  asm volatile("global_store_dword %0, %1, %2 offset:%3" :: "v"(voff), "v"(x), "s"(p), "n"(OFF) : "memory");
+}
+template <int N>
+__device__ __forceinline__ void ep_wait(const float (&a)[8]) {
+  asm volatile("s_waitcnt vmcnt(%0)" :: "n"(N), "v"(a[0]), "v"(a[1]), "v"(a[2]), "v"(a[3]), "v"(a[4]), "v"(a[5]), "v"(a[6]),
+               "v"(a[7]) : "memory");
+  __builtin_amdgcn_sched_barrier(0);
+}
+template <int N>
+__device__ __forceinline__ void ep_wait(const float (&a)[8], const float (&b)[8]) {
+  asm volatile("s_waitcnt vmcnt(%0)" :: "n"(N), "v"(a[0]), "v"(a[1]), "v"(a[2]), "v"(a[3]), "v"(a[4]), "v"(a[5]), "v"(a[6]),
+               "v"(a[7]), "v"(b[0]), "v"(b[1]), "v"(b[2]), "v"(b[3]), "v"(b[4]), "v"(b[5]), "v"(b[6]), "v"(b[7]) : "memory");
+  __builtin_amdgcn_sched_barrier(0);
+}
+template <int N>
+__device__ __forceinline__ void ep_wait(float a, float b) {
+  asm volatile("s_waitcnt vmcnt(%0)" :: "n"(N), "v"(a), "v"(b) : "memory");
+  __builtin_amdgcn_sched_barrier(0);
+}
+__device__ __forceinline__ float ep_row(float rowvec, int addr) {
+  return __int_as_float(__builtin_amdgcn_ds_bpermute(addr, __float_as_int(rowvec)));
+}
+template <class T>
+__device__ __forceinline__ T* ep_uniform(T* p) {
+  const uint64_t a = reinterpret_cast<uint64_t>(p);
+  const uint32_t lo = __builtin_amdgcn_readfirstlane((uint32_t)a), hi = __builtin_amdgcn_readfirstlane((uint32_t)(a >> 32));
+  return reinterpret_cast<T*>(((uint64_t)hi << 32) | lo);
+}
+
+template <int EPI>
+__device__ __forceinline__ void split_epilogue_interior(const GemmArgs& g, f32x16 (&acc)[2][2], int bz, int m0, int n0,
+                                                        int wm, int wn, int li, int lh) {
+  constexpr bool BIAS = EPI & EP_BIAS, MAP = EPI & EP_MAP, ZOUT = EPI & EP_ZOUT, SILU = EPI & EP_SILU, ZMUL = EPI & EP_ZMUL,
+                 RES = EPI & EP_RES, GATE = EPI & EP_GATE;
+  static_assert(!(GATE && !RES) && !(ZMUL && (SILU || ZOUT)), "no such epilogue");
+  constexpr int NT = MAP + ZMUL + RES, I_MAP = 0, I_ZM = MAP, I_RES = MAP + ZMUL;
+  static_assert(NT <= 2, "a third operand tensor needs a third ep_wait");
+  constexpr int L = 8 * NT, S = 8 * (1 + ZOUT);
+  const int wrow = __builtin_amdgcn_readfirstlane(m0 + wm * 64), wcol = __builtin_amdgcn_readfirstlane(n0 + wn * 64);
+  const int64_t ld = g.ldc, tile = (int64_t)wrow * ld + wcol;
+  float* const Cs = ep_uniform(g.C + (int64_t)bz * g.c_bs + tile);
+  float* const zos = ZOUT ? ep_uniform(g.zout + (int64_t)bz * g.zout_bs + tile) : nullptr;
+  const float* const mps = MAP ? ep_uniform(g.map + tile) : nullptr;
+  const float* const zms = ZMUL ? ep_uniform(g.zmul + (int64_t)bz * g.zmul_bs + tile) : nullptr;
+  const float* const rss = RES ? ep_uniform(g.res + (int64_t)bz * g.res_bs + tile) : nullptr;
+  const uint32_t voff = ((uint32_t)(4 * lh) * (uint32_t)ld + (uint32_t)li) * 4u;
+  const int radr = 16 * lh;
+  auto rowof = [](int gi, int q) constexpr { return (gi >> 2) * 32 + (q & 3) + 8 * (2 * ((gi >> 1) & 1) + (q >> 2)); };
+
+  float bv = 0.f, gv = 0.f;
+  float buf[2][NT ? NT : 1][8];
+  auto issue = [&](auto G) __attribute__((always_inline)) {
+    constexpr int gi = decltype(G)::value, OFF = (gi & 1) * 128;
+#pragma unroll
+    for (int q = 0; q < 8; ++q) {
+      const int64_t ro = (int64_t)rowof(gi, q) * ld;
+      if constexpr (MAP) ep_load<OFF>(buf[gi & 1][I_MAP][q], voff, mps + ro);
+      if constexpr (ZMUL) ep_load<OFF>(buf[gi & 1][I_ZM][q], voff, zms + ro);
+      if constexpr (RES) ep_load<OFF>(buf[gi & 1][I_RES][q], voff, rss + ro);
+    }
+  };
+  float br[8], gr[8];
+  if constexpr (BIAS) ep_load<0>(bv, (uint32_t)(32 * lh + li) * 4u, ep_uniform(g.bias + wrow));
+  if constexpr (GATE) ep_load<0>(gv, (uint32_t)(32 * lh + li) * 4u, ep_uniform(g.gate + wrow));
+  if constexpr (NT > 0) issue(std::integral_constant<int, 0>{});
+  __builtin_amdgcn_sched_barrier(0);
+
+  auto group = [&](auto G) __attribute__((always_inline)) {
+    constexpr int gi = decltype(G)::value, tm = gi >> 2, h = (gi >> 1) & 1, tn = gi & 1, OFF = tn * 128, b = gi & 1;
+    if constexpr (NT > 0 && gi < 7) {
+      issue(std::integral_constant<int, gi + 1>{});
+      __builtin_amdgcn_sched_barrier(0);
+    }
+    if constexpr (gi == 0 && (BIAS || GATE)) {
+      ep_wait<NT ? 2 * L : 0>(bv, gv);
+      if constexpr (GATE) gv = gate_sigmoid(gv);
+    }
+    if constexpr (tn == 0 && (BIAS || GATE)) {
+#pragma unroll
+      for (int q = 0; q < 8; ++q) {
+        if constexpr (BIAS) br[q] = ep_row(bv, radr + 4 * rowof(gi, q));
+        if constexpr (GATE) gr[q] = ep_row(gv, radr + 4 * rowof(gi, q));
+      }
+      __builtin_amdgcn_sched_barrier(0);
+    }
+    constexpr int YOUNGER = (gi < 7 ? L : 0) + (gi > 0 ? S : 0);
+    if constexpr (NT == 1) ep_wait<YOUNGER>(buf[b][0]);
+    if constexpr (NT == 2) ep_wait<YOUNGER>(buf[b][0], buf[b][1]);
+    float v[8];
+#pragma unroll
+    for (int q = 0; q < 8; ++q) v[q] = acc[tm][tn][8 * h + q];
+    if constexpr (BIAS) {
+#pragma unroll
+      for (int q = 0; q < 8; ++q) v[q] += br[q];
+    }
+    if constexpr (MAP) {
+#pragma unroll
+      for (int q = 0; q < 8; ++q) v[q] += buf[b][I_MAP][q];
+    }
+    if constexpr (ZOUT) {
+#pragma unroll
+      for (int q = 0; q < 8; ++q) ep_store<OFF>(v[q], voff, zos + (int64_t)rowof(gi, q) * ld);
+    }
+    if constexpr (ZMUL) {
+#pragma unroll
+      for (int q = 0; q < 8; ++q) v[q] *= act_grad(buf[b][I_ZM][q], PARADIS_ACT_SILU);
+    } else if constexpr (SILU) {
+#pragma unroll
+      for (int q = 0; q < 8; ++q) v[q] = act_apply(v[q], PARADIS_ACT_SILU);
+    }
+    if constexpr (RES) {
+#pragma unroll
+      for (int q = 0; q < 8; ++q) {
+        const float r = buf[b][I_RES][q];
+        if constexpr (GATE) v[q] = fmaf(gr[q], v[q] - r, r);
+        else v[q] += r;
+      }
+    }
+#pragma unroll
+    for (int q = 0; q < 8; ++q) ep_store<OFF>(v[q], voff, Cs + (int64_t)rowof(gi, q) * ld);
+    __builtin_amdgcn_sched_barrier(0);
+  };
+  group(std::integral_constant<int, 0>{}); group(std::integral_constant<int, 1>{});
+  group(std::integral_constant<int, 2>{}); group(std::integral_constant<int, 3>{});
+  group(std::integral_constant<int, 4>{}); group(std::integral_constant<int, 5>{});
+  group(std::integral_constant<int, 6>{}); group(std::integral_constant<int, 7>{});
+}
+
 typedef float f32x4 __attribute__((ext_vector_type(4)));
-template <int NP>
+template <int NP, int A32 = 0>
 __global__ void __launch_bounds__(256, 3)
 pw_gemm_wgrad_split_kernel(GemmArgs g) {
   extern __shared__ __attribute__((aligned(16))) float lds[];
+  static_assert(A32 == 0 || NP == 3, "the scalar-base loads exist in the bf16x3 instantiation only");
+  constexpr bool SADDR = A32 != 0 && SPLIT_WGRAD_SADDR;
+  constexpr bool SIGN_COPIES = NP == 3 && SPLIT_SIGN_LOOPS_WGRAD && SPLIT_SIGNED_WGRAD;
+  constexpr bool ROWSUM_COPIES = NP == 3 && SPLIT_WGRAD_ROWSUM_LOOP;
   constexpr int SIMGP = simgp(NP);
   u32x4* img = reinterpret_cast<u32x4*>(lds);
   const int tid = threadIdx.x, lane = tid & 63, wave = tid >> 6;
@@ -534,30 +714,33 @@
     const int q = nwg >> 3, r = nwg & 7, xcd = id & 7;
     L = (xcd < r ? xcd * (q + 1) : r * (q + 1) + (xcd - r) * q) + (id >> 3);
   }
-  const int mt = L % MT, nt = (L / MT) % NT, bz = L / (MT * NT);
+  int mt = L % MT, nt = (L / MT) % NT, bz = L / (MT * NT);
+  if constexpr (SIGN_COPIES || ROWSUM_COPIES || SADDR) {
+    mt = __builtin_amdgcn_readfirstlane(mt); nt = __builtin_amdgcn_readfirstlane(nt); bz = __builtin_amdgcn_readfirstlane(bz);
+  }
   const int m0 = mt * BM, n0 = nt * BN;
   const int KT = g.K / SBK;
   const int64_t total = (int64_t)g.inner * KT;
-  const int t_begin = (int)(total * bz / g.nbatch);
-  const int T = (int)(total * (bz + 1) / g.nbatch) - t_begin;
-
-  const int srow = tid >> 1, sh = tid & 1;
-  const float* Ag = g.A + (int64_t)min(m0 + srow, g.M - 1) * g.lda + sh * 8;
-  const float* Bg = g.B + (int64_t)min(n0 + srow, g.N - 1) * g.ldb + sh * 8;
-
-  int f_ib = t_begin / KT, f_kt = t_begin - f_ib * KT;
+  int t_begin = (int)(total * bz / g.nbatch);
+  int T = (int)(total * (bz + 1) / g.nbatch) - t_begin;
+  if constexpr (SADDR) {
+    t_begin = __builtin_amdgcn_readfirstlane(t_begin);
+    T = __builtin_amdgcn_readfirstlane(T);
+  }
+
+  int f_ib0 = t_begin / KT, f_kt0 = t_begin - f_ib0 * KT;
+  const float* sa0 = nullptr;
+  const float* sb0 = nullptr;
+  int64_t wrap_a = 0, wrap_b = 0;
+  if constexpr (SADDR) {
+    f_ib0 = __builtin_amdgcn_readfirstlane(f_ib0);
+    f_kt0 = __builtin_amdgcn_readfirstlane(f_kt0);
+    sa0 = ep_uniform(g.A + (int64_t)m0 * g.lda + (int64_t)f_ib0 * g.a_is + (int64_t)f_kt0 * SBK);
+    sb0 = ep_uniform(g.B + (int64_t)n0 * g.ldb + (int64_t)f_ib0 * g.b_is + (int64_t)f_kt0 * SBK);
+    wrap_a = g.a_is - (int64_t)KT * SBK;
+    wrap_b = g.b_is - (int64_t)KT * SBK;
+  }
   struct Regs { f32x4 a0, a1, b0, b1; };
-  const f32x4 zero4 = {0.f, 0.f, 0.f, 0.f};
-  Regs r0{zero4, zero4, zero4, zero4}, r1 = r0;
-  auto fetch = [&](Regs& r) __attribute__((always_inline)) {
-    const float* a = Ag + (int64_t)f_ib * g.a_is + (int64_t)f_kt * SBK;
-    const float* b = Bg + (int64_t)f_ib * g.b_is + (int64_t)f_kt * SBK;
-    asm volatile("global_load_dwordx4 %0, %1, off" : "=&v"(r.a0) : "v"(a) : "memory");
-    asm volatile("global_load_dwordx4 %0, %1, off offset:16" : "=&v"(r.a1) : "v"(a) : "memory");
-    asm volatile("global_load_dwordx4 %0, %1, off" : "=&v"(r.b0) : "v"(b) : "memory");
-    asm volatile("global_load_dwordx4 %0, %1, off offset:16" : "=&v"(r.b1) : "v"(b) : "memory");
-    if (++f_kt == KT) { f_kt = 0; ++f_ib; }
-  };
 #define USE_R(r, N) do { asm volatile("s_waitcnt vmcnt(" #N ")" :: "v"(r.a0), "v"(r.a1), "v"(r.b0), "v"(r.b1) : "memory"); \
                          __builtin_amdgcn_sched_barrier(0); } while (0)
   const bool do_rowsum = g.rowsum != nullptr && nt == 0;
@@ -569,17 +752,24 @@
   }
   const uint32_t slab_flip = (SPLIT_SIGNED_WGRAD && (bz & 1)) ? 0x80000000u : 0u;
   if constexpr (NP == 2) sc_a = __uint_as_float(__float_as_uint(sc_a) ^ slab_flip);
-  auto split_store = [&](const Regs& r, int st, bool keep) __attribute__((always_inline)) {
+  auto split_store = [&](auto SG, auto RS, const Regs& r, u32x4* o0, int st, bool keep) __attribute__((always_inline)) {
+    constexpr int sg = decltype(SG)::value, rsm = decltype(RS)::value;
     const float xa[8] = {r.a0.x, r.a0.y, r.a0.z, r.a0.w, r.a1.x, r.a1.y, r.a1.z, r.a1.w};
     const float xb[8] = {r.b0.x, r.b0.y, r.b0.z, r.b0.w, r.b1.x, r.b1.y, r.b1.z, r.b1.w};
-    const float add = ((xa[0] + xa[1]) + (xa[2] + xa[3])) + ((xa[4] + xa[5]) + (xa[6] + xa[7]));
-    rs += keep ? add : 0.f;
-    u32x4* o = img + st * 2 * SIMGP + sh * SCHP + srow;
+    if constexpr (rsm != 0) {
+      const float add = ((xa[0] + xa[1]) + (xa[2] + xa[3])) + ((xa[4] + xa[5]) + (xa[6] + xa[7]));
+      rs += keep ? add : 0.f;
+    }
+    u32x4* o = o0 + st * 2 * SIMGP;
     if constexpr (NP == 3) {
       u32x4 ha, ma, la, hb, mb, lb;
-      float xs[8];
-      flip8(xs, xa, slab_flip);
-      split8(xs, ha, ma, la);
+      if constexpr (sg == 2) {
+        float xs[8];
+        flip8(xs, xa, slab_flip);
+        split8(xs, ha, ma, la);
+      } else {
+        split8s<sg == 1>(xa, ha, ma, la);
+      }
       split8(xb, hb, mb, lb);
       o[0] = ha; o[2 * SCHP] = ma; o[4 * SCHP] = la;
       o += SIMGP;
@@ -600,59 +790,121 @@
   };
 
   f32x16 acc[2][2];
-#pragma unroll
-  for (int i = 0; i < 2; ++i)
-#pragma unroll
-    for (int j = 0; j < 2; ++j)
-#pragma unroll
-      for (int r = 0; r < 16; ++r) acc[i][j][r] = 0.f;
-
-  if (T > 0) {
-    fetch(r0);
-    if (T > 1) { fetch(r1); USE_R(r0, 4); } else { USE_R(r0, 0); }
-    split_store(r0, 0, do_rowsum);
-  }
-  asm volatile("s_waitcnt lgkmcnt(0)\n\ts_barrier" ::: "memory");
-
-  auto step = [&](int t, int cur, Regs& rload, Regs& rsplit) __attribute__((always_inline)) {
-    const u32x4* As = img + cur * 2 * SIMGP + lh * SCHP + wm * 64 + li;
-    const u32x4* Bs = img + (cur * 2 + 1) * SIMGP + lh * SCHP + wn * 64 + li;
-    SplitFrags<NP> f;
-    split_tile_read<NP, 2 * SCHP, 2 * SCHP>(As, Bs, f);
-    __builtin_amdgcn_sched_barrier(0);
-    if (t + 2 < T) { fetch(rload); USE_R(rsplit, 4); }
-    else USE_R(rsplit, 0);
-    split_tile_mfma<NP>(f, acc);
-    split_store(rsplit, cur ^ 1, do_rowsum && t + 1 < T);
-    if constexpr (NP > 1) {
-#pragma unroll
-    for (int i = 0; i < (NP == 3 ? 24 : 12); ++i) {
-      __builtin_amdgcn_sched_group_barrier(0x008, 1, 0);
-      __builtin_amdgcn_sched_group_barrier(0x002, 5, 0);
-    }
+  auto run = [&](auto SG, auto RS) __attribute__((always_inline)) {
+    constexpr int sg = decltype(SG)::value, rsm = decltype(RS)::value;
+    const bool rsum = rsm == 2 ? do_rowsum : true;
+    float zero = 0.f;
+    if constexpr (sg != 2 || rsm != 2) asm volatile("" : "+v"(zero));
+#pragma unroll
+    for (int i = 0; i < 2; ++i)
+#pragma unroll
+      for (int j = 0; j < 2; ++j)
+#pragma unroll
+        for (int r = 0; r < 16; ++r) acc[i][j][r] = zero;
+    int ot = tid;
+    if constexpr (sg != 2 || rsm != 2) asm volatile("" : "+v"(ot));
+    const int lwm = (ot >> 7) & 1, lwn = (ot >> 6) & 1, lli = ot & 31, llh = (ot >> 5) & 1;
+    const int srow = ot >> 1, sh = ot & 1;
+    u32x4* const o0 = img + sh * SCHP + srow;
+    const float* const Ag = SADDR ? nullptr : g.A + (int64_t)min(m0 + srow, g.M - 1) * g.lda + sh * 8;
+    const float* const Bg = SADDR ? nullptr : g.B + (int64_t)min(n0 + srow, g.N - 1) * g.ldb + sh * 8;
+    const uint32_t voa = ((uint32_t)min(srow, g.M - 1 - m0) * (uint32_t)g.lda + (uint32_t)(sh * 8)) * 4u;
+    const uint32_t vob = ((uint32_t)min(srow, g.N - 1 - n0) * (uint32_t)g.ldb + (uint32_t)(sh * 8)) * 4u;
+    int f_ib = f_ib0, f_kt = f_kt0;
+    const float* sa = sa0;
+    const float* sb = sb0;
+    const f32x4 zero4 = {0.f, 0.f, 0.f, 0.f};
+    Regs r0{zero4, zero4, zero4, zero4}, r1 = r0;
+    auto fetch = [&](Regs& r) __attribute__((always_inline)) {
+      if constexpr (SADDR) {
+        asm volatile("global_load_dwordx4 %0, %1, %2" : "=&v"(r.a0) : "v"(voa), "s"(sa) : "memory");
+        asm volatile("global_load_dwordx4 %0, %1, %2 offset:16" : "=&v"(r.a1) : "v"(voa), "s"(sa) : "memory");
+        asm volatile("global_load_dwordx4 %0, %1, %2" : "=&v"(r.b0) : "v"(vob), "s"(sb) : "memory");
+        asm volatile("global_load_dwordx4 %0, %1, %2 offset:16" : "=&v"(r.b1) : "v"(vob), "s"(sb) : "memory");
+        sa += SBK; sb += SBK;
+        if (++f_kt == KT) { f_kt = 0; sa += wrap_a; sb += wrap_b; }
+      } else {
+        const float* a = Ag + (int64_t)f_ib * g.a_is + (int64_t)f_kt * SBK;
+        const float* b = Bg + (int64_t)f_ib * g.b_is + (int64_t)f_kt * SBK;
+        asm volatile("global_load_dwordx4 %0, %1, off" : "=&v"(r.a0) : "v"(a) : "memory");
+        asm volatile("global_load_dwordx4 %0, %1, off offset:16" : "=&v"(r.a1) : "v"(a) : "memory");
+        asm volatile("global_load_dwordx4 %0, %1, off" : "=&v"(r.b0) : "v"(b) : "memory");
+        asm volatile("global_load_dwordx4 %0, %1, off offset:16" : "=&v"(r.b1) : "v"(b) : "memory");
+        if (++f_kt == KT) { f_kt = 0; ++f_ib; }
+      }
+    };
+    if (T > 0) {
+      fetch(r0);
+      if (T > 1) { fetch(r1); USE_R(r0, 4); } else { USE_R(r0, 0); }
+      split_store(SG, RS, r0, o0, 0, rsum);
     }
     asm volatile("s_waitcnt lgkmcnt(0)\n\ts_barrier" ::: "memory");
+
+    auto step = [&](int t, int cur, Regs& rload, Regs& rsplit) __attribute__((always_inline)) {
+      const u32x4* As = img + cur * 2 * SIMGP + llh * SCHP + lwm * 64 + lli;
+      const u32x4* Bs = img + (cur * 2 + 1) * SIMGP + llh * SCHP + lwn * 64 + lli;
+      SplitFrags<NP> f;
+      split_tile_read<NP, 2 * SCHP, 2 * SCHP>(As, Bs, f);
+      __builtin_amdgcn_sched_barrier(0);
+      if (t + 2 < T) { fetch(rload); USE_R(rsplit, 4); }
+      else USE_R(rsplit, 0);
+      split_tile_mfma<NP>(f, acc);
+      split_store(SG, RS, rsplit, o0, cur ^ 1, rsum && t + 1 < T);
+      if constexpr (NP > 1) {
+#pragma unroll
+        for (int i = 0; i < (NP == 3 ? 24 : 12); ++i) {
+          __builtin_amdgcn_sched_group_barrier(0x008, 1, 0);
+          __builtin_amdgcn_sched_group_barrier(0x002, 5, 0);
+        }
+      }
+      asm volatile("s_waitcnt lgkmcnt(0)\n\ts_barrier" ::: "memory");
+    };
+    for (int t = 0; t < T; t += 2) {
+      step(t, 0, r0, r1);
+      if (t + 1 < T) step(t + 1, 1, r1, r0);
+    }
+    if (sg == 1 || (sg == 2 && slab_flip)) {
+#pragma unroll
+      for (int i = 0; i < 2; ++i)
+#pragma unroll
+        for (int j = 0; j < 2; ++j)
+#pragma unroll
+          for (int r = 0; r < 16; ++r) acc[i][j][r] = -acc[i][j][r];
+    }
   };
-  for (int t = 0; t < T; t += 2) {
-    step(t, 0, r0, r1);
-    if (t + 1 < T) step(t + 1, 1, r1, r0);
+  {
+    using std::integral_constant;
+    constexpr integral_constant<int, SIGN_COPIES ? 0 : 2> plain;
+    constexpr integral_constant<int, SIGN_COPIES ? 1 : 2> negated;
+    constexpr integral_constant<int, ROWSUM_COPIES ? 0 : 2> no_sums;
+    constexpr integral_constant<int, ROWSUM_COPIES ? 1 : 2> sums;
+    const bool neg = SIGN_COPIES && slab_flip != 0, with_sums = ROWSUM_COPIES && do_rowsum;
+    if (with_sums) {
+      if (neg) run(negated, sums); else run(plain, sums);
+    } else {
+      if (neg) run(negated, no_sums); else run(plain, no_sums);
+    }
   }
 #undef USE_R
   if (do_rowsum) {
+    int t = tid;
+    if constexpr (SIGN_COPIES || ROWSUM_COPIES) asm volatile("" : "+v"(t));
     rs += __shfl_xor(rs, 1, 64);
-    const int m = m0 + srow;
-    if (sh == 0 && m < g.M) g.rowsum[(int64_t)bz * g.M + m] = rs;
-  }
-  if (slab_flip) {
-#pragma unroll
-    for (int i = 0; i < 2; ++i)
-#pragma unroll
-      for (int j = 0; j < 2; ++j)
-#pragma unroll
-        for (int r = 0; r < 16; ++r) acc[i][j][r] = -acc[i][j][r];
+    const int m = m0 + (t >> 1);
+    if ((t & 1) == 0 && m < g.M) g.rowsum[(int64_t)bz * g.M + m] = rs;
   }
   if constexpr (NP == 2) split_unscale(acc, inv_a, inv_b);
-  gemm_epilogue(g, acc, bz, m0, n0, wm, wn, li, lh);
+  if constexpr (SIGN_COPIES || ROWSUM_COPIES || (NP == 3 && SPLIT_WGRAD_EPILOGUE)) {
+    int t = tid;
+    asm volatile("" : "+v"(t));
+    const int ew = __builtin_amdgcn_readfirstlane((t >> 6) & 3), ewm = ew >> 1, ewn = ew & 1, eli = t & 31, elh = (t >> 5) & 1;
+    if (NP == 3 && SPLIT_WGRAD_EPILOGUE && !g.generic_epilogue && m0 + BM <= g.M && n0 + BN <= g.N)
+      split_epilogue_interior<EP_ON>(g, acc, bz, m0, n0, ewm, ewn, eli, elh);
+    else
+      gemm_epilogue(g, acc, bz, m0, n0, ewm, ewn, eli, elh);
+  } else {
+    gemm_epilogue(g, acc, bz, m0, n0, wm, wn, li, lh);
+  }
 }
 
 typedef void (*GemmKernel)(GemmArgs);
diff --git a/paradis_model_amd/csrc/gemm_split.hip b/paradis_model_amd/csrc/gemm_split.hip
--- a/paradis_model_amd/csrc/gemm_split.hip
+++ b/paradis_model_amd/csrc/gemm_split.hip
@@ -95,142 +95,6 @@
     u32x4* o = out + tile * simg(2) + half * SCH + row;
     o[0] = h; o[2 * SCH] = l;
   }
-}
-
-enum : int { EP_ON = 1, EP_BIAS = 2, EP_MAP = 4, EP_ZOUT = 8, EP_SILU = 16, EP_ZMUL = 32, EP_RES = 64, EP_GATE = 128 };
-
-template <int OFF>
-__device__ __forceinline__ void ep_load(float& x, uint32_t voff, const float* p) {
-  asm volatile("global_load_dword %0, %1, %2 offset:%3" : "=&v"(x) : "v"(voff), "s"(p), "n"(OFF) : "memory");
-}
-template <int OFF>
-__device__ __forceinline__ void ep_store(float x, uint32_t voff, float* p) {
-  asm volatile("global_store_dword %0, %1, %2 offset:%3" :: "v"(voff), "v"(x), "s"(p), "n"(OFF) : "memory");
-}
-template <int N>
-__device__ __forceinline__ void ep_wait(const float (&a)[8]) {
-  asm volatile("s_waitcnt vmcnt(%0)" :: "n"(N), "v"(a[0]), "v"(a[1]), "v"(a[2]), "v"(a[3]), "v"(a[4]), "v"(a[5]), "v"(a[6]),
-               "v"(a[7]) : "memory");
-  __builtin_amdgcn_sched_barrier(0);
-}
-template <int N>
-__device__ __forceinline__ void ep_wait(const float (&a)[8], const float (&b)[8]) {
-  asm volatile("s_waitcnt vmcnt(%0)" :: "n"(N), "v"(a[0]), "v"(a[1]), "v"(a[2]), "v"(a[3]), "v"(a[4]), "v"(a[5]), "v"(a[6]),
-               "v"(a[7]), "v"(b[0]), "v"(b[1]), "v"(b[2]), "v"(b[3]), "v"(b[4]), "v"(b[5]), "v"(b[6]), "v"(b[7]) : "memory");
-  __builtin_amdgcn_sched_barrier(0);
-}
-template <int N>
-__device__ __forceinline__ void ep_wait(float a, float b) {
-  asm volatile("s_waitcnt vmcnt(%0)" :: "n"(N), "v"(a), "v"(b) : "memory");
-  __builtin_amdgcn_sched_barrier(0);
-}
-__device__ __forceinline__ float ep_row(float rowvec, int addr) {
-  return __int_as_float(__builtin_amdgcn_ds_bpermute(addr, __float_as_int(rowvec)));
-}
-template <class T>
-__device__ __forceinline__ T* ep_uniform(T* p) {
-  const uint64_t a = reinterpret_cast<uint64_t>(p);
-  const uint32_t lo = __builtin_amdgcn_readfirstlane((uint32_t)a), hi = __builtin_amdgcn_readfirstlane((uint32_t)(a >> 32));
-  return reinterpret_cast<T*>(((uint64_t)hi << 32) | lo);
-}
-
-template <int EPI>
-__device__ __forceinline__ void split_epilogue_interior(const GemmArgs& g, f32x16 (&acc)[2][2], int bz, int m0, int n0,
-                                                        int wm, int wn, int li, int lh) {
-  constexpr bool BIAS = EPI & EP_BIAS, MAP = EPI & EP_MAP, ZOUT = EPI & EP_ZOUT, SILU = EPI & EP_SILU, ZMUL = EPI & EP_ZMUL,
-                 RES = EPI & EP_RES, GATE = EPI & EP_GATE;
-  static_assert(!(GATE && !RES) && !(ZMUL && (SILU || ZOUT)), "no such epilogue");
-  constexpr int NT = MAP + ZMUL + RES, I_MAP = 0, I_ZM = MAP, I_RES = MAP + ZMUL;
-  static_assert(NT <= 2, "a third operand tensor needs a third ep_wait");
-  constexpr int L = 8 * NT, S = 8 * (1 + ZOUT);
-  const int wrow = __builtin_amdgcn_readfirstlane(m0 + wm * 64), wcol = __builtin_amdgcn_readfirstlane(n0 + wn * 64);
-  const int64_t ld = g.ldc, tile = (int64_t)wrow * ld + wcol;
-  float* const Cs = ep_uniform(g.C + (int64_t)bz * g.c_bs + tile);
-  float* const zos = ZOUT ? ep_uniform(g.zout + (int64_t)bz * g.zout_bs + tile) : nullptr;
-  const float* const mps = MAP ? ep_uniform(g.map + tile) : nullptr;
-  const float* const zms = ZMUL ? ep_uniform(g.zmul + (int64_t)bz * g.zmul_bs + tile) : nullptr;
-  const float* const rss = RES ? ep_uniform(g.res + (int64_t)bz * g.res_bs + tile) : nullptr;
-  const uint32_t voff = ((uint32_t)(4 * lh) * (uint32_t)ld + (uint32_t)li) * 4u;
-  const int radr = 16 * lh;
-  auto rowof = [](int gi, int q) constexpr { return (gi >> 2) * 32 + (q & 3) + 8 * (2 * ((gi >> 1) & 1) + (q >> 2)); };
-
-  float bv = 0.f, gv = 0.f;
-  float buf[2][NT ? NT : 1][8];
-  auto issue = [&](auto G) __attribute__((always_inline)) {
-    constexpr int gi = decltype(G)::value, OFF = (gi & 1) * 128;
-#pragma unroll
-    for (int q = 0; q < 8; ++q) {
-      const int64_t ro = (int64_t)rowof(gi, q) * ld;
-      if constexpr (MAP) ep_load<OFF>(buf[gi & 1][I_MAP][q], voff, mps + ro);
-      if constexpr (ZMUL) ep_load<OFF>(buf[gi & 1][I_ZM][q], voff, zms + ro);
-      if constexpr (RES) ep_load<OFF>(buf[gi & 1][I_RES][q], voff, rss + ro);
-    }
-  };
-  float br[8], gr[8];
-  if constexpr (BIAS) ep_load<0>(bv, (uint32_t)(32 * lh + li) * 4u, ep_uniform(g.bias + wrow));
-  if constexpr (GATE) ep_load<0>(gv, (uint32_t)(32 * lh + li) * 4u, ep_uniform(g.gate + wrow));
-  if constexpr (NT > 0) issue(std::integral_constant<int, 0>{});
-  __builtin_amdgcn_sched_barrier(0);
-
-  auto group = [&](auto G) __attribute__((always_inline)) {
-    constexpr int gi = decltype(G)::value, tm = gi >> 2, h = (gi >> 1) & 1, tn = gi & 1, OFF = tn * 128, b = gi & 1;
-    if constexpr (NT > 0 && gi < 7) {
-      issue(std::integral_constant<int, gi + 1>{});
-      __builtin_amdgcn_sched_barrier(0);
-    }
-    if constexpr (gi == 0 && (BIAS || GATE)) {
-      ep_wait<NT ? 2 * L : 0>(bv, gv);
-      if constexpr (GATE) gv = gate_sigmoid(gv);
-    }
-    if constexpr (tn == 0 && (BIAS || GATE)) {
-#pragma unroll
-      for (int q = 0; q < 8; ++q) {
-        if constexpr (BIAS) br[q] = ep_row(bv, radr + 4 * rowof(gi, q));
-        if constexpr (GATE) gr[q] = ep_row(gv, radr + 4 * rowof(gi, q));
-      }
-      __builtin_amdgcn_sched_barrier(0);
-    }
-    constexpr int YOUNGER = (gi < 7 ? L : 0) + (gi > 0 ? S : 0);
-    if constexpr (NT == 1) ep_wait<YOUNGER>(buf[b][0]);
-    if constexpr (NT == 2) ep_wait<YOUNGER>(buf[b][0], buf[b][1]);
-    float v[8];
-#pragma unroll
-    for (int q = 0; q < 8; ++q) v[q] = acc[tm][tn][8 * h + q];
-    if constexpr (BIAS) {
-#pragma unroll
-      for (int q = 0; q < 8; ++q) v[q] += br[q];
-    }
-    if constexpr (MAP) {
-#pragma unroll
-      for (int q = 0; q < 8; ++q) v[q] += buf[b][I_MAP][q];
-    }
-    if constexpr (ZOUT) {
-#pragma unroll
-      for (int q = 0; q < 8; ++q) ep_store<OFF>(v[q], voff, zos + (int64_t)rowof(gi, q) * ld);
-    }
-    if constexpr (ZMUL) {
-#pragma unroll
-      for (int q = 0; q < 8; ++q) v[q] *= act_grad(buf[b][I_ZM][q], PARADIS_ACT_SILU);
-    } else if constexpr (SILU) {
-#pragma unroll
-      for (int q = 0; q < 8; ++q) v[q] = act_apply(v[q], PARADIS_ACT_SILU);
-    }
-    if constexpr (RES) {
-#pragma unroll
-      for (int q = 0; q < 8; ++q) {
-        const float r = buf[b][I_RES][q];
-        if constexpr (GATE) v[q] = fmaf(gr[q], v[q] - r, r);
-        else v[q] += r;
-      }
-    }
-#pragma unroll
-    for (int q = 0; q < 8; ++q) ep_store<OFF>(v[q], voff, Cs + (int64_t)rowof(gi, q) * ld);
-    __builtin_amdgcn_sched_barrier(0);
-  };
-  group(std::integral_constant<int, 0>{}); group(std::integral_constant<int, 1>{});
-  group(std::integral_constant<int, 2>{}); group(std::integral_constant<int, 3>{});
-  group(std::integral_constant<int, 4>{}); group(std::integral_constant<int, 5>{});
-  group(std::integral_constant<int, 6>{}); group(std::integral_constant<int, 7>{});
 }
 
 #ifndef SPLIT_ASTAGES_F16
@@ -381,7 +245,10 @@
     const int q = nwg >> 3, r = nwg & 7, xcd = id & 7;
     L = (xcd < r ? xcd * (q + 1) : r * (q + 1) + (xcd - r) * q) + (id >> 3);
   }
-  const int mt = L % MT, nt2 = (L / MT) % NT2, bz = L / (MT * NT2);
+  int mt = L % MT, nt2 = (L / MT) % NT2, bz = L / (MT * NT2);
+  if constexpr (NP == 3 && SPLIT_SIGN_LOOPS_FWD && SPLIT_SIGNED) {
+    mt = __builtin_amdgcn_readfirstlane(mt); nt2 = __builtin_amdgcn_readfirstlane(nt2); bz = __builtin_amdgcn_readfirstlane(bz);
+  }
   const bool live = NSUB * nt2 + sub < NT;
   const int nt = min(NSUB * nt2 + sub, NT - 1);
   const int m0 = mt * BM, n0 = nt * BN;
@@ -417,19 +284,23 @@
 
   const uint32_t flip = split_flip_mask(ltid & 127);
   if constexpr (NP == 2) sc_b = __uint_as_float(__float_as_uint(sc_b) ^ flip);
-  float xb[2][8] = {};
   auto issueA = [&](int t) __attribute__((always_inline)) {
     if (doA)
       __builtin_amdgcn_global_load_lds((gbl_ptr_t)(Ag + (int64_t)t * SIMG), (lds_ptr_t)(img + (2 * NSUB + t % SA) * SIMG + wave * 64), 16, 0, 0);
     if (doA2)
       __builtin_amdgcn_global_load_lds((gbl_ptr_t)(Ag + (int64_t)t * SIMG + 512), (lds_ptr_t)(img + (2 * NSUB + t % SA) * SIMG + 512 + wave * 64), 16, 0, 0);
   };
-  auto split_store = [&](const float (&x)[8], u32x4* o) __attribute__((always_inline)) {
+  auto split_store = [&](auto SG, const float (&x)[8], u32x4* o) __attribute__((always_inline)) {
+    constexpr int sg = decltype(SG)::value;
     if constexpr (NP == 3) {
       u32x4 h, m, l;
-      float xs[8];
-      flip8(xs, x, flip);
-      split8(xs, h, m, l);
+      if constexpr (sg == 2) {
+        float xs[8];
+        flip8(xs, x, flip);
+        split8(xs, h, m, l);
+      } else {
+        split8s<sg == 1>(x, h, m, l);
+      }
       o[0] = h; o[2 * SCH] = m; o[4 * SCH] = l;
     } else {
       u32x4 h, l;
@@ -453,74 +324,85 @@
   u32x4* const Bst = img + sub * 2 * SIMG + bh * SCH + (ltid & 127);
 
   f32x16 acc[2][2];
-#pragma unroll
-  for (int i = 0; i < 2; ++i)
-#pragma unroll
-    for (int j = 0; j < 2; ++j)
-#pragma unroll
-      for (int r = 0; r < 16; ++r) acc[i][j][r] = 0.f;
-
-  for (int u = 0; u < DA && u < T; ++u) issueA(u);
-  fetchB(0, xb[0]);
-  USE_X(xb[0], 0);
-  if (T > 1) fetchB(1, xb[1]);
-  split_store(xb[0], Bst);
-  if (T > 1) asm volatile("s_waitcnt vmcnt(8) lgkmcnt(0)\n\ts_barrier" ::: "memory");
-  else asm volatile("s_waitcnt vmcnt(0) lgkmcnt(0)\n\ts_barrier" ::: "memory");
-  auto step = [&](int t, int cur, float (&xload)[8], float (&xsplit)[8]) __attribute__((always_inline)) {
-    const u32x4* As = img + (2 * NSUB + t % SA) * SIMG + lh * SCH + wm * 64 + li;
-    const u32x4* Bs = img + (sub * 2 + cur) * SIMG + lh * SCH + wn * 64 + li;
-    const bool dmaA = t + DA < T, ldB = t + 2 < T;
-    if (dmaA) issueA(t + DA);
-    if (ldB) fetchB(t + 2, xload);
-    if (dmaA && ldB && doA2) USE_X(xsplit, 10);
-    else if (dmaA && ldB && doA) USE_X(xsplit, 9);
-    else if (ldB) USE_X(xsplit, 8);
-    else USE_X(xsplit, 0);
-    if constexpr (NP == 3) {
-      auto mfma_block = [&]() __attribute__((always_inline)) {
-        u32x4 a[3][2], b[2];
-#pragma unroll
-        for (int pl = 0; pl < 3; ++pl) { a[pl][0] = As[pl * 2 * SCH]; a[pl][1] = As[pl * 2 * SCH + 32]; }
-#pragma unroll
-        for (int pb = 2; pb >= 0; --pb) {
-          b[0] = Bs[pb * 2 * SCH]; b[1] = Bs[pb * 2 * SCH + 32];
-#pragma unroll
-          for (int pa = 2 - pb; pa >= 0; --pa)
-#pragma unroll
-            for (int tm = 0; tm < 2; ++tm)
-#pragma unroll
-              for (int tn = 0; tn < 2; ++tn) SPLIT_MFMA(a[pa][tm], b[tn], acc[tm][tn]);
+
+  auto run = [&](auto SG) __attribute__((always_inline)) {
+    float zero = 0.f;
+    if constexpr (decltype(SG)::value != 2) asm volatile("" : "+v"(zero));
+#pragma unroll
+    for (int i = 0; i < 2; ++i)
+#pragma unroll
+      for (int j = 0; j < 2; ++j)
+#pragma unroll
+        for (int r = 0; r < 16; ++r) acc[i][j][r] = zero;
+    float xb[2][8] = {};
+    for (int u = 0; u < DA && u < T; ++u) issueA(u);
+    fetchB(0, xb[0]);
+    USE_X(xb[0], 0);
+    if (T > 1) fetchB(1, xb[1]);
+    split_store(SG, xb[0], Bst);
+    if (T > 1) asm volatile("s_waitcnt vmcnt(8) lgkmcnt(0)\n\ts_barrier" ::: "memory");
+    else asm volatile("s_waitcnt vmcnt(0) lgkmcnt(0)\n\ts_barrier" ::: "memory");
+    auto step = [&](int t, int cur, float (&xload)[8], float (&xsplit)[8]) __attribute__((always_inline)) {
+      const u32x4* As = img + (2 * NSUB + t % SA) * SIMG + lh * SCH + wm * 64 + li;
+      const u32x4* Bs = img + (sub * 2 + cur) * SIMG + lh * SCH + wn * 64 + li;
+      const bool dmaA = t + DA < T, ldB = t + 2 < T;
+      if (dmaA) issueA(t + DA);
+      if (ldB) fetchB(t + 2, xload);
+      if (dmaA && ldB && doA2) USE_X(xsplit, 10);
+      else if (dmaA && ldB && doA) USE_X(xsplit, 9);
+      else if (ldB) USE_X(xsplit, 8);
+      else USE_X(xsplit, 0);
+      if constexpr (NP == 3) {
+        auto mfma_block = [&]() __attribute__((always_inline)) {
+          u32x4 a[3][2], b[2];
+#pragma unroll
+          for (int pl = 0; pl < 3; ++pl) { a[pl][0] = As[pl * 2 * SCH]; a[pl][1] = As[pl * 2 * SCH + 32]; }
+#pragma unroll
+          for (int pb = 2; pb >= 0; --pb) {
+            b[0] = Bs[pb * 2 * SCH]; b[1] = Bs[pb * 2 * SCH + 32];
+#pragma unroll
+            for (int pa = 2 - pb; pa >= 0; --pa)
+#pragma unroll
+              for (int tm = 0; tm < 2; ++tm)
+#pragma unroll
+                for (int tn = 0; tn < 2; ++tn) SPLIT_MFMA(a[pa][tm], b[tn], acc[tm][tn]);
+          }
+        };
+#if SPLIT_STAGGER
+        if (sub == 1) split_store(SG, xsplit, Bst + (cur ^ 1) * SIMG);
+        __builtin_amdgcn_sched_barrier(0);
+        mfma_block();
+        __builtin_amdgcn_sched_barrier(0);
+        if (sub == 0) split_store(SG, xsplit, Bst + (cur ^ 1) * SIMG);
+#else
+        mfma_block();
+        split_store(SG, xsplit, Bst + (cur ^ 1) * SIMG);
+#endif
+      } else {
+        SplitFrags<NP> f;
+        split_tile_read<NP, 2 * SCH, 2 * SCH>(As, Bs, f);
+        split_tile_mfma<NP>(f, acc);
+        split_store(SG, xsplit, Bst + (cur ^ 1) * SIMG);
+        __builtin_amdgcn_sched_group_barrier(0x100, 4 * NP, 0);
+#pragma unroll
+        for (int i = 0; i < 12; ++i) {
+          __builtin_amdgcn_sched_group_barrier(0x008, 1, 0);
+          __builtin_amdgcn_sched_group_barrier(0x002, 2, 0);
         }
-      };
-#if SPLIT_STAGGER
-      if (sub == 1) split_store(xsplit, Bst + (cur ^ 1) * SIMG);
-      __builtin_amdgcn_sched_barrier(0);
-      mfma_block();
-      __builtin_amdgcn_sched_barrier(0);
-      if (sub == 0) split_store(xsplit, Bst + (cur ^ 1) * SIMG);
-#else
-      mfma_block();
-      split_store(xsplit, Bst + (cur ^ 1) * SIMG);
-#endif
-    } else {
-      SplitFrags<NP> f;
-      split_tile_read<NP, 2 * SCH, 2 * SCH>(As, Bs, f);
-      split_tile_mfma<NP>(f, acc);
-      split_store(xsplit, Bst + (cur ^ 1) * SIMG);
-      __builtin_amdgcn_sched_group_barrier(0x100, 4 * NP, 0);
-#pragma unroll
-      for (int i = 0; i < 12; ++i) {
-        __builtin_amdgcn_sched_group_barrier(0x008, 1, 0);
-        __builtin_amdgcn_sched_group_barrier(0x002, 2, 0);
       }
-    }
-    if (dmaA && ldB) asm volatile("s_waitcnt vmcnt(8) lgkmcnt(0)\n\ts_barrier" ::: "memory");
-    else asm volatile("s_waitcnt vmcnt(0) lgkmcnt(0)\n\ts_barrier" ::: "memory");
-  };
-  for (int t = 0; t < T; t += 2) {
-    step(t, 0, xb[0], xb[1]);
-    if (t + 1 < T) step(t + 1, 1, xb[1], xb[0]);
+      if (dmaA && ldB) asm volatile("s_waitcnt vmcnt(8) lgkmcnt(0)\n\ts_barrier" ::: "memory");
+      else asm volatile("s_waitcnt vmcnt(0) lgkmcnt(0)\n\ts_barrier" ::: "memory");
+    };
+    for (int t = 0; t < T; t += 2) {
+      step(t, 0, xb[0], xb[1]);
+      if (t + 1 < T) step(t + 1, 1, xb[1], xb[0]);
+    }
+  };
+  if constexpr (NP == 3 && SPLIT_SIGN_LOOPS_FWD && SPLIT_SIGNED) {
+    if (__builtin_amdgcn_readfirstlane((ltid >> 6) & 1)) run(std::integral_constant<int, 1>{});
+    else run(std::integral_constant<int, 0>{});
+  } else {
+    run(std::integral_constant<int, 2>{});
   }
 #undef USE_X
   if (live) {
@@ -567,8 +449,9 @@
 constexpr GemmKernelEntry SPLIT[2] = {{&pw_gemm_split_kernel<2>, split_lds(2)}, {&pw_gemm_split_kernel<3>, split_lds(3)}};
 constexpr GemmKernelEntry SPLIT_WIDE[2] = {{&pw_gemm_split_wide_kernel<SPLIT_WIDE_NSUB, 2>, split_wide_lds(SPLIT_WIDE_NSUB, 2)},
                                            {&pw_gemm_split_wide_kernel<SPLIT_WIDE_NSUB, 3>, split_wide_lds(SPLIT_WIDE_NSUB, 3)}};
-constexpr GemmKernelEntry SPLIT_WGRAD[2] = {{&pw_gemm_wgrad_split_kernel<2>, split_lds_wgrad(2)},
-                                            {&pw_gemm_wgrad_split_kernel<3>, split_lds_wgrad(3)}};
+constexpr GemmKernelEntry SPLIT_WGRAD[3] = {{&pw_gemm_wgrad_split_kernel<2>, split_lds_wgrad(2)},
+                                            {&pw_gemm_wgrad_split_kernel<3>, split_lds_wgrad(3)},
+                                            {&pw_gemm_wgrad_split_kernel<3, 1>, split_lds_wgrad(3)}};
 #define EPI_SETS(X)                                                                                                       \
   X(EP_ON) X(EP_ON | EP_ZMUL)                                                                         \
   X(EP_ON | EP_BIAS) X(EP_ON | EP_BIAS | EP_RES) X(EP_ON | EP_BIAS | EP_RES | EP_GATE)                      \
@@ -678,9 +561,18 @@
   return launch_entry(SPLIT, np - 2, once, "pw_gemm(split)", MT * NT * d.nbatch, 256, st, d);
 }
 
+bool split_wgrad_a32(const GemmArgs& g) {
+  constexpr int64_t LIM = (int64_t)1 << 22;
+  return SPLIT_WGRAD_SADDR && g.lda >= 0 && g.lda < LIM && g.ldb >= 0 && g.ldb < LIM;
+}
+
 int pd_split_launch_wgrad(const GemmArgs& g, const WgradPlan& p, hipStream_t st) {
   static PerDeviceOnce once;
-  return launch_entry(SPLIT_WGRAD, p.kind == WgradKind::F16x2 ? 0 : 1, once, "pw_gemm_wgrad(split)", p.grid, p.block, st, g, p.lds);
+  if (p.kind == WgradKind::F16x2) return launch_entry(SPLIT_WGRAD, 0, once, "pw_gemm_wgrad(split)", p.grid, p.block, st, g, p.lds);
+  GemmArgs d = g;
+  const char* e = getenv("PARADIS_GEMM_EPILOGUE");
+  d.generic_epilogue = (e && strcmp(e, "generic") == 0) || d.ldc >= (1 << 26);
+  return launch_entry(SPLIT_WGRAD, split_wgrad_a32(d) ? 2 : 1, once, "pw_gemm_wgrad(split)", p.grid, p.block, st, d, p.lds);
 }
 
 int64_t pd_split_image_chunks(int M, int K, int np) { return split_image_chunks(M, K, np); }
```

Result: faster. 220.4 samples/s, median of 6 (+2.9%).
